# DakeQQ/Text-to-Speech-TTS-ONNX

Measured on AMD Instinct MI355X. Metric: audio_seconds_per_second, higher is better.
Workload: dtype f32

## Files before the change

include/mi355tts.h:

```cpp
#ifndef MI355TTS_H
#define MI355TTS_H

#include <stdint.h>

#ifdef __cplusplus
extern "C" {
#endif

enum { MI_F32 = 0, MI_F16 = 1, MI_BF16 = 2 };
enum { MI_HOST = 0, MI_DEVICE = 1 };
enum { MI_OK = 0, MI_EINVAL = -1, MI_EHIP = -2, MI_ENOMEM = -3, MI_ESTATE = -4 };

typedef struct mi_bigvgan mi_bigvgan;
typedef struct mi_f5 mi_f5;

int         mi_init(int device);
int         mi_device_count(void);
const char* mi_last_error(void);
const char* mi_version(void);

int64_t     mi_bigvgan_param_count(const int32_t* cfg, int n_cfg);
mi_bigvgan* mi_bigvgan_create(const int32_t* cfg, int n_cfg, const float* weights, int64_t n_weights,
                              int dtype, int device);
mi_bigvgan* mi_bigvgan_create_mem(const int32_t* cfg, int n_cfg, const float* weights, int64_t n_weights,
// ... 99 lines not shown
                                          int penalty_range, float* repeat_penality, int32_t* tokens, float* hidden, int cap,
                                          int32_t* n_out, int mem, const float* temperature, const int32_t* top_k,
                                          const float* top_p, const uint64_t* seeds);
int         mi_gpt_sample_logits(const float* logits, const float* pen, int rows, int codes, const float* temperature,
                                 const int32_t* top_k, const float* top_p, const uint64_t* seeds, const int64_t* positions,
                                 int32_t* tokens, float* u_out, float* prob_out, int mem);

int         mi_gpt_generate_beam(mi_gpt* h, int nb, const float* prompts, const int32_t* prompt_rows, const int32_t* max_new,
                                 const int32_t* stop_ids, int n_stop, float repeat_value, int penalty_range,
                                 float* repeat_penality, int num_beams, int32_t* tokens, float* hidden, int cap, int32_t* n_out,
                                 float* scores, int mem);
int         mi_gpt_beam_select(const float* logits, const float* pen, const float* prev_scores, int groups, int beams, int codes,
                               int first, int32_t* parents, int32_t* tokens, float* scores, int mem);

int         mi_gpt_generate_beam_pool(mi_gpt* h, int nb, const float* prompts, const int32_t* prompt_rows, const int32_t* max_new,
                                      const int32_t* stop_ids, int n_stop, float repeat_value, int penalty_range,
                                      const float* repeat_penality, int num_beams, float length_penalty, int early_stopping,
                                      const float* temperature, const int32_t* top_k, const float* top_p, const uint64_t* seeds,
                                      int32_t* tokens, float* hidden, int cap, int32_t* n_out, float* scores, int mem);
int         mi_gpt_beam_pool_select(const float* logits, const float* pen, const float* prev_scores, int beams, int codes, int n,
                                    int max_new, const int32_t* stop_ids, int n_stop, float* pool_scores, int32_t* pool_finished,
                                    int32_t* open, float length_penalty, int early_stopping, const float* temperature,
                                    const int32_t* top_k, const float* top_p, const uint64_t* seed, int32_t* cand, float* cand_acc,
                                    int32_t* cand_stop, int32_t* parents, int32_t* tokens, float* scores, int32_t* pool_src,
                                    int32_t* done, int mem);

int         mi_gpt_attn_decode(const float* qkv, const float* kc, const float* vc, int dtype, int heads, int max_seq, int nslots,
                               const int32_t* hist, float* out, int mem);
int         mi_gpt_attn_decode_beam(const float* qkv, const float* kc, const float* vc, int dtype, int heads, int max_seq,
                                    int nslots, const int32_t* hist, const int32_t* ndec, int beams, const int32_t* anc, float* out,
                                    int mem);
int         mi_gpt_attn_prompt(const float* qkv, const float* kc, const float* vc, int dtype, int heads, int max_seq, int hist,
                               int rows, int flag, float* out, int mem);
int         mi_gpt_attn_prompt_packed(const float* qkv, const float* kc, const float* vc, int dtype, int heads, int max_seq,
                                      int nslots, const int32_t* segs, int nseg, int total, float* out, int mem);

int         mi_gpt_linear_decode(const float* w, const float* bias, const float* x, int dtype, int n, int k, const float* ln_w,
                                 const float* ln_b, const float* pre_w, const float* pre_b, float* pre_out, const float* res,
                                 int act, int out_f32, int qkv, int hist, int max_seq, float* kc, float* vc, float* out, int mem);
int         mi_gpt_linear_batch(const float* w, const float* bias, const float* x, const float* x_dead, int dtype, int n, int k,
                                int nb, const float* res, int act, int out_f32, int qkv, const int32_t* hist, int max_seq,
                                float* kc, float* vc, float* out, int mem);
int         mi_gpt_linear_batch_rows(int nb);
int         mi_gpt_linear_decode_q8(const uint8_t* q, const float* scale, const uint8_t* zp, const float* bias, const float* x,
                                    int dtype, int n, int k, const float* ln_w, const float* ln_b, const float* pre_w,
                                    const float* pre_b, float* pre_out, const float* res, int act, int out_f32, int qkv, int hist,
                                    int max_seq, float* kc, float* vc, float* out, int mem);
int         mi_gpt_linear_batch_q8(const uint8_t* q, const float* scale, const uint8_t* zp, const float* bias, const float* x,
                                   const float* x_dead, int dtype, int n, int k, int nb, const float* res, int act, int out_f32,
                                   int qkv, const int32_t* hist, int max_seq, float* kc, float* vc, float* out, int mem);

int         mi_gpt_generate_queue(mi_gpt* h, int n, const float* prompts, const int32_t* prompt_rows, const int32_t* max_new,
                                  const int32_t* stop_ids, int n_stop, float repeat_value, int penalty_range,
                                  int32_t* tokens, float* hidden, int cap, int32_t* n_out, int mem,
                                  const float* temperature, const int32_t* top_k, const float* top_p, const uint64_t* seeds,
                                  int32_t* stats );

int         mi_gpt_queue_begin(mi_gpt* h, int n, const float* prompts, const int32_t* prompt_rows, const int32_t* max_new,
                               const int32_t* stop_ids, int n_stop, float repeat_value, int penalty_range, int32_t* tokens,
                               float* hidden, int cap, int mem, const float* temperature, const int32_t* top_k, const float* top_p,
                               const uint64_t* seeds);
int         mi_gpt_queue_advance(mi_gpt* h, int32_t* count , int32_t* done , int32_t* finished ,
                                 int32_t* stats );
int         mi_gpt_queue_end(mi_gpt* h);

int         mi_gpt_generate_queue_beam(mi_gpt* h, int n, const float* prompts, const int32_t* prompt_rows, const int32_t* max_new,
                                       const int32_t* stop_ids, int n_stop, float repeat_value, int penalty_range, int num_beams,
                                       int32_t* tokens, float* hidden, int cap, int32_t* n_out, float* scores ,
                                       int mem, int32_t* stats );
int         mi_gpt_queue_begin_beam(mi_gpt* h, int n, const float* prompts, const int32_t* prompt_rows, const int32_t* max_new,
                                    const int32_t* stop_ids, int n_stop, float repeat_value, int penalty_range, int num_beams,
                                    int32_t* tokens, float* hidden, int cap, float* scores , int mem);

int         mi_gpt_queue_schedule(int n, const int32_t* prompt_rows, const int32_t* max_new, const int32_t* lengths, int slots,
                                  int max_seq, int beams, int32_t* steps, int32_t* n_passes, int32_t* pass_of ,
                                  int32_t* unit_of );

int         mi_gpt_bench_pick(mi_gpt* h, int nb, int iters, const float* temperature, const int32_t* top_k, const float* top_p,
                              double* us);

int         mi_bench_conv_gemm(int dtype, int B, int T, int Cin, int N, int taps, int dil, int with_res, int iters,
                               double* ms);

#define MI_GEMM_PLAN_INTS 10
int         mi_conv_gemm_plan(int dtype, int B, int T, int Cin, int N, int taps, int dil, int with_res, int cus,
                              int32_t* plans , int* n_launches);

int64_t     mi_indextts_cond_param_count(const int32_t* cfg, int n_cfg);
mi_cond*    mi_indextts_cond_create(const int32_t* cfg, int n_cfg, const float* weights, int64_t n_weights, int device);
void        mi_indextts_cond_destroy(mi_cond* h);
int         mi_indextts_cond_run(mi_cond* h, const int16_t* audio, int64_t L, float* conds, float* conds_latent, float* mel,
                                 int mem);

int         mi_set_option(const char* key, int64_t value);
int         mi_get_option(const char* key, int64_t* value);
int         mi_device_pci_bus_id(int device, char* buf, int cap);

int         mi_prof_enable(int family_mask);
int         mi_prof_reset(void);
int         mi_prof_get(const char* family, double* ms, int64_t* launches, double* bytes, double* flops);
int         mi_prof_kernel_count(void);
int         mi_prof_kernel_get(int index, char* name, int name_cap, char* family, int family_cap, double* ms,
                               int64_t* launches, double* bytes, double* flops);

#ifdef __cplusplus
}
#endif
#endif
```

text-to-speech-tts-onnx_amd/csrc/capi.hip:

```cpp
#include "common.h"
#include "bigvgan.h"
#include "f5.h"
#include "gpt.h"
#include "gpt_queue.h"
#include "gpt_pool.h"
#include "cond.h"
#include <algorithm>
#include <memory>
#include <mutex>
#include <exception>

using namespace mi;

struct mi_bigvgan { BigVGAN* impl; std::mutex mu; };
struct mi_f5 { F5* impl; std::mutex mu; };
struct mi_gpt { Gpt* impl; std::mutex mu; std::unique_ptr<GptQueue> session; };
struct mi_cond { Cond* impl; std::mutex mu; };

template <typename F> static int guard(F&& f, bool exclusive = false) {
    try {
        options_init();
        std::shared_lock<std::shared_mutex> rd(option_lock(), std::defer_lock);
        std::unique_lock<std::shared_mutex> wr(option_lock(), std::defer_lock);
        if (exclusive) wr.lock(); else rd.lock();
// ... 218 lines not shown
    return guard([&] {
        MI_REQUIRE(x && w && y && B > 0 && Cin > 0 && Cout > 0 && T > 0 && k > 0 && dilation > 0 && groups > 0 && padding >= 0,
                   "mi_conv1d: bad arguments");
        unit_conv1d(x, B, Cin, T, w, bias, Cout, k, dilation, padding, groups, dtype, y);
    });
}

int mi_conv_transpose1d(const float* x, int B, int Cin, int T, const float* w, const float* bias, int Cout, int k,
                        int stride, int padding, int dtype, float* y) {
    return guard([&] {
        MI_REQUIRE(x && w && y && B > 0 && Cin > 0 && Cout > 0 && T > 0, "mi_conv_transpose1d: bad arguments");
        unit_conv_transpose1d(x, B, Cin, T, w, bias, Cout, k, stride, padding, dtype, y);
    });
}

int64_t mi_f5_param_count(const int32_t* cfg_i, int n_i, const float* cfg_f, int n_f) {
    int64_t n = -1;
    int rc = guard([&] { n = f5_param_count(parse_f5_cfg(cfg_i, n_i, cfg_f, n_f)); });
    return rc == MI_OK ? n : (int64_t)rc;
}

mi_f5* mi_f5_create(const int32_t* cfg_i, int n_i, const float* cfg_f, int n_f, const float* weights, int64_t n_weights,
                    int dtype, int device) {
    mi_f5* h = nullptr;
    int rc = guard([&] {
        MI_REQUIRE(weights != nullptr, "mi_f5_create: null weights");
        F5Cfg c = parse_f5_cfg(cfg_i, n_i, cfg_f, n_f);
        F5* impl = new F5(c, weights, n_weights, dtype, device);
        h = new mi_f5; h->impl = impl;
    });
    return rc == MI_OK ? h : nullptr;
}

mi_f5* mi_f5_create_mem(const int32_t* cfg_i, int n_i, const float* cfg_f, int n_f, const float* weights, int64_t n_weights,
                        int dtype, int device, int mem) {
    mi_f5* h = nullptr;
    int rc = guard([&] {
        MI_REQUIRE(weights != nullptr && (mem == MI_HOST || mem == MI_DEVICE), "mi_f5_create_mem: null weights / bad mem kind");
        F5Cfg c = parse_f5_cfg(cfg_i, n_i, cfg_f, n_f);
        F5* impl = new F5(c, weights, n_weights, dtype, device, mem);
        h = new mi_f5; h->impl = impl;
    });
    return rc == MI_OK ? h : nullptr;
}

void mi_f5_destroy(mi_f5* h) {
    if (!h) return;
    delete h->impl;
    delete h;
}

struct F5Recover {
    F5* e; int n;
    explicit F5Recover(F5* e_) : e(e_), n(std::uncaught_exceptions()) {}
    ~F5Recover() { if (std::uncaught_exceptions() > n) e->recover(); }
};
#define F5_CHECK(h, mem, name)                                                     \
    MI_REQUIRE((h) && (h)->impl, name ": null handle");                            \
    std::lock_guard<std::mutex> lk_((h)->mu);                                      \
    F5Recover rec_((h)->impl);                                                     \
    ArithScope arith_((h)->impl->arith);                                           \
    MI_REQUIRE((mem) == MI_HOST || (mem) == MI_DEVICE, name ": bad mem kind")

int mi_f5_tables(mi_f5* h, float* time_expand, float* delta_t) {
    return guard([&] {
        MI_REQUIRE(h && h->impl, "mi_f5_tables: null handle");
        std::lock_guard<std::mutex> lk_(h->mu);
        F5& e = *h->impl;
        if (time_expand) std::memcpy(time_expand, e.h_time_expand.data(), e.h_time_expand.size() * 4);
        if (delta_t) std::memcpy(delta_t, e.h_delta.data(), e.h_delta.size() * 4);
    });
}

int64_t mi_f5_info(mi_f5* h, const char* key) {
    int64_t v = -1;
    int rc = guard([&] {
        MI_REQUIRE(h && h->impl && key, "mi_f5_info: null handle / key");
        std::lock_guard<std::mutex> lk_(h->mu);
        F5& e = *h->impl;
        ArithScope as(e.arith);
        const std::string k(key);
        if (k == "f32_arithmetic") v = e.dtype != MI_F32 ? -1 : !gemm_x3_enabled() ? ARITH_NATIVE : (gemm_x3p_enabled() ? e.np : ARITH_BF16X3);
        else if (k == "saturation_events") v = e.sat_events;
        else if (k == "adaln_fold") v = (e.fold_built && e.cfg.ln_fold != 0) ? 1 : 0;
        else if (k == "attn_v_rows") v = attention_kv_layout(0, e.dtype, true).v_rows;
        else MI_REQUIRE(false, "mi_f5_info: unknown key");
    });
    return rc == MI_OK ? v : (int64_t)rc;
}

int mi_f5_preprocess(mi_f5* h, const int16_t* audio, int64_t L, const int32_t* text_ids, int64_t T, int64_t max_duration,
                     const float* noise_in, uint64_t seed, float* noise, float* rope_cos, float* rope_sin,
                     float* cat_mel_text, float* cat_mel_text_drop, int64_t* ref_signal_len, int mem) {
    return guard([&] {
        F5_CHECK(h, mem, "mi_f5_preprocess");
        F5& e = *h->impl;
        MI_REQUIRE(max_duration > 0 && max_duration <= e.cfg.max_len && T >= 0 && T < (1 << 20) && L > 0 && L < (1L << 31),
                   "mi_f5_preprocess: sizes");
        const int N = (int)max_duration;
        const int R = e.preprocess(1, audio, L, text_ids, (int)T, N, noise_in, seed, mem);
        hipStream_t s = e.stream;
        const size_t cd = e.cfg.cond_dim(), D = e.cfg.dim_head;
        copy_out(noise, e.d_noise.p, (size_t)N * e.cfg.mel * 4, mem, s);
        copy_out(rope_cos, e.rope_cos.p, (size_t)N * D * 4, mem, s);
        copy_out(rope_sin, e.rope_sin.p, (size_t)N * D * 4, mem, s);
        copy_out(cat_mel_text, e.d_cmt.p, (size_t)N * cd * 4, mem, s);
        copy_out(cat_mel_text_drop, e.d_cmtd.p, (size_t)N * cd * 4, mem, s);
        MI_HIP(hipStreamSynchronize(s));
        e.finish_call();
        if (ref_signal_len) *ref_signal_len = R;
    });
}

int mi_f5_transformer_step(mi_f5* h, float* noise, const float* cmt, const float* cmtd, int U, int64_t N,
                           int32_t* time_step, int fuse, int mem) {
    return guard([&] {
        F5_CHECK(h, mem, "mi_f5_transformer_step");
        MI_REQUIRE(noise && cmt && cmtd && time_step && fuse >= 1 && U >= 1 && N > 0, "mi_f5_transformer_step: bad arguments");
        F5& e = *h->impl;
        f5_run_checked(e, [&] {
            e.load_cond(noise, cmt, cmtd, U, (int)N, mem);
            e.build_cat_cond(U, (int)N);
            e.steps(U, (int)N, *time_step, fuse);
            MI_HIP(hipStreamSynchronize(e.stream));
        });
        copy_out(noise, e.d_noise.p, (size_t)U * N * e.cfg.mel * 4, mem, e.stream);
        MI_HIP(hipStreamSynchronize(e.stream));
        e.finish_call();
        *time_step += fuse;
    });
}

int mi_f5_sample(mi_f5* h, float* noise, const float* cmt, const float* cmtd, int U, int64_t N, int k0, int n_steps, int mem) {
    return guard([&] {
        F5_CHECK(h, mem, "mi_f5_sample");
        MI_REQUIRE(noise && cmt && cmtd && U >= 1 && N > 0, "mi_f5_sample: bad arguments");
        F5& e = *h->impl;
        f5_run_checked(e, [&] {
            e.load_cond(noise, cmt, cmtd, U, (int)N, mem);
            e.build_cat_cond(U, (int)N);
            e.steps(U, (int)N, k0, n_steps);
            MI_HIP(hipStreamSynchronize(e.stream));
        });
        copy_out(noise, e.d_noise.p, (size_t)U * N * e.cfg.mel * 4, mem, e.stream);
        MI_HIP(hipStreamSynchronize(e.stream));
        e.finish_call();
    });
}

int mi_f5_dit_eval(mi_f5* h, const float* noise, const float* cmt, const float* cmtd, int U, int64_t N, int k, float* pred, int mem) {
    return guard([&] {
        F5_CHECK(h, mem, "mi_f5_dit_eval");
        MI_REQUIRE(noise && cmt && cmtd && pred && U >= 1 && N > 0, "mi_f5_dit_eval: bad arguments");
        F5& e = *h->impl;
        f5_run_checked(e, [&] {
            e.load_cond(noise, cmt, cmtd, U, (int)N, mem);
            e.build_cat_cond(U, (int)N);
            e.dit_eval(U, (int)N, k);
            MI_HIP(hipStreamSynchronize(e.stream));
        });
        copy_out(pred, e.pred_rows(U, (int)N), (size_t)2 * U * N * e.cfg.mel * 4, mem, e.stream);
        MI_HIP(hipStreamSynchronize(e.stream));
        e.finish_call();
    });
}

// ... 1094 lines not shown
        const void* xd = ln_w ? (const void*)u.f32(x, k) : u.typed(x, 1, k, dtype);
        void* kd = qkv ? u.typed(kc, (long)(nc / 64), 64, dtype) : nullptr;
        void* vd = qkv ? u.typed(vc, (long)(nc / 64), 64, dtype) : nullptr;
        void* od = u.nan_out(n, odt);
        float* pd = pre_w ? (float*)u.nan_out(k, MI_F32) : nullptr;
        const int* st = u.state(&hist, 1, 1);
        launch_gpt_gemv(l, xd, u.f32(ln_w, k), u.f32(ln_b, k), u.f32(pre_w, k), u.f32(pre_b, k), pd, od, odt, act, u.f32(res, n), kd,
                        vd, st, qkv ? max_seq : 1, u.s);
        u.give(out, od, n, odt);
        if (pd) u.give(pre_out, pd, k, MI_F32);
        if (qkv) { u.give(kc, kd, nc, dtype); u.give(vc, vd, nc, dtype); }
        MI_HIP(hipStreamSynchronize(u.s));
    });
}

int mi_gpt_linear_decode(const float* w, const float* bias, const float* x, int dtype, int n, int k, const float* ln_w,
                         const float* ln_b, const float* pre_w, const float* pre_b, float* pre_out, const float* res, int act,
                         int out_f32, int qkv, int hist, int max_seq, float* kc, float* vc, float* out, int mem) {
    return linear_decode_unit("mi_gpt_linear_decode", w, LinQ8{nullptr, nullptr, nullptr}, bias, x, dtype, n, k, ln_w, ln_b, pre_w, pre_b,
                              pre_out, res, act, out_f32, qkv, hist, max_seq, kc, vc, out, mem);
}

int mi_gpt_linear_decode_q8(const uint8_t* q, const float* scale, const uint8_t* zp, const float* bias, const float* x, int dtype, int n,
                            int k, const float* ln_w, const float* ln_b, const float* pre_w, const float* pre_b, float* pre_out,
                            const float* res, int act, int out_f32, int qkv, int hist, int max_seq, float* kc, float* vc, float* out,
                            int mem) {
    if (!q) return guard([&] { MI_REQUIRE(false, "mi_gpt_linear_decode_q8: null argument"); });
    return linear_decode_unit("mi_gpt_linear_decode_q8", nullptr, LinQ8{q, scale, zp}, bias, x, dtype, n, k, ln_w, ln_b, pre_w, pre_b,
                              pre_out, res, act, out_f32, qkv, hist, max_seq, kc, vc, out, mem);
}

static int linear_batch_unit(const std::string& who, const float* w, const LinQ8& q8, const float* bias, const float* x,
                             const float* x_dead, int dtype, int n, int k, int nb, const float* res, int act, int out_f32, int qkv,
                             const int32_t* hist, int max_seq, float* kc, float* vc, float* out, int mem) {
    return guard([&] {
        LinUnit u(who, dtype, mem);
        MI_REQUIRE(x && out, who + ": null argument");
        MI_REQUIRE(nb >= 1 && nb <= GPT_MAX_BATCH, who + ": nb must be in [1, 64]");
        MI_REQUIRE(n >= 1 && n <= (1 << 20) && k >= 1 && k <= 16384, who + ": n must be in [1, 2^20], k in [1, 16384]");
        MI_REQUIRE(act == ACT_NONE || act == ACT_GELU_TANH, who + ": act must be 0 or 1 (gelu_new)");
        if (qkv) {
            MI_REQUIRE(n % 3 == 0 && n == 3 * k && k % 64 == 0, who + ": qkv needs n == 3 * k (a multiple of 3), k a multiple of 64");
            MI_REQUIRE(kc && vc && hist, who + ": qkv needs kc, vc and hist");
            MI_REQUIRE(max_seq >= 1 && max_seq <= 8192, who + ": max_seq must be in [1, 8192]");
            for (int b = 0; b < nb; ++b) MI_REQUIRE(hist[b] >= 0 && hist[b] <= max_seq, who + ": hist must be in [0, max_seq]");
        }
        const int odt = out_f32 ? MI_F32 : dtype, P = gpt_padded_rows(nb);
        const size_t sstride = qkv ? (size_t)k * max_seq : 0, nc = (size_t)nb * sstride;
        const GptLin l = lin_unit_weights(u, who, w, q8, bias, dtype, n, k);
        char* xd = (char*)u.typed(x, nb, k, dtype, P);
        const size_t row = (size_t)k * dtype_size(dtype);
        if (x_dead) {
            const float* dead = u.f32(x_dead, k);
            for (int b = nb; b < P; ++b) launch_copy2d(dead, k, xd + b * row, k, 1, k, dtype, u.s);
        } else if (P > nb) {
            MI_HIP(hipMemsetAsync(xd + nb * row, 0, (P - nb) * row, u.s));
        }
        void* kd = qkv ? u.typed(kc, (long)(nc / 64), 64, dtype) : nullptr;
        void* vd = qkv ? u.typed(vc, (long)(nc / 64), 64, dtype) : nullptr;
        void* od = u.nan_out((size_t)P * n, odt);
        const int* st = u.state(qkv ? hist : nullptr, nb, P);
        launch_gpt_gemv_b(l, xd, nb, P, od, odt, act, u.f32(res, (size_t)nb * n), kd, vd, st, qkv ? max_seq : 1, sstride, u.s);
        u.give(out, od, (size_t)P * n, odt);
        if (qkv) { u.give(kc, kd, nc, dtype); u.give(vc, vd, nc, dtype); }
        MI_HIP(hipStreamSynchronize(u.s));
    });
}

int mi_gpt_linear_batch(const float* w, const float* bias, const float* x, const float* x_dead, int dtype, int n, int k, int nb,
                        const float* res, int act, int out_f32, int qkv, const int32_t* hist, int max_seq, float* kc, float* vc,
                        float* out, int mem) {
    return linear_batch_unit("mi_gpt_linear_batch", w, LinQ8{nullptr, nullptr, nullptr}, bias, x, x_dead, dtype, n, k, nb, res, act, out_f32,
                             qkv, hist, max_seq, kc, vc, out, mem);
}

int mi_gpt_linear_batch_q8(const uint8_t* q, const float* scale, const uint8_t* zp, const float* bias, const float* x,
                           const float* x_dead, int dtype, int n, int k, int nb, const float* res, int act, int out_f32, int qkv,
                           const int32_t* hist, int max_seq, float* kc, float* vc, float* out, int mem) {
    if (!q) return guard([&] { MI_REQUIRE(false, "mi_gpt_linear_batch_q8: null argument"); });
    return linear_batch_unit("mi_gpt_linear_batch_q8", nullptr, LinQ8{q, scale, zp}, bias, x, x_dead, dtype, n, k, nb, res, act, out_f32,
                             qkv, hist, max_seq, kc, vc, out, mem);
}

extern "C++" {
enum { BG_X, BG_W, BG_BIAS, BG_OUT, BG_RES, BG_W3, BG_XP, BG_W3P, BG_SK_WS, BG_SK_FLAGS, BG_COUNT };
template <typename F> static ConvGemm bench_gemm(int dtype, int B, int T, int Cin, int N, int taps, int dil, int with_res, F&& buf) {
    const size_t es = dtype_size(dtype), nx = (size_t)B * T * Cin, nw = (size_t)N * taps * Cin, no = (size_t)B * T * N;
    ConvGemm p;
    p.dtype = dtype; p.x = buf(BG_X, nx * es); p.w = buf(BG_W, nw * es); p.bias = (const float*)buf(BG_BIAS, (size_t)N * 4); p.out = buf(BG_OUT, no * es);
    p.res = with_res ? buf(BG_RES, no * es) : nullptr;
    p.B = B; p.T_in = T; p.M = T; p.N = N; p.Cin = Cin; p.taps = taps; p.dil = dil; p.pad = (taps * dil - dil) / 2;
    p.x_bstride = (long)T * Cin; p.x_rstride = Cin; p.out_bstride = (long)T * N; p.out_rstride = N;
    p.sk_slots = 1024; p.sk_ws = (float*)buf(BG_SK_WS, (size_t)p.sk_slots * 128 * 128 * 4); p.sk_flags = (int*)buf(BG_SK_FLAGS, (size_t)p.sk_slots * 4);
    if (dtype == MI_F32 && taps == 1 && gemm_x3_enabled()) p.w3 = buf(BG_W3, (size_t)3 * nw * 2);
    if (p.w3 && gemm_x3p_enabled() && N % 128 == 0 && Cin % 32 == 0 && p.pad == 0) {
        p.np = x3p_planes();
        p.xp = buf(BG_XP, (size_t)x3p_bytes((long)B * T, Cin, p.np)); p.w3p = buf(BG_W3P, (size_t)x3p_bytes(N, Cin, p.np));
    }
    return p;
}
}

int mi_conv_gemm_plan(int dtype, int B, int T, int Cin, int N, int taps, int dil, int with_res, int cus, int32_t* plans, int* n_launches) {
    return guard([&] {
        MI_REQUIRE(plans && n_launches && (dtype == MI_F32 || dtype == MI_F16 || dtype == MI_BF16) && B > 0 && T > 0 && Cin > 0 && N > 0 && taps > 0 && dil > 0 && cus > 0,
                   "mi_conv_gemm_plan: bad arguments");
        ConvGemm p = bench_gemm(dtype, B, T, Cin, N, taps, dil, with_res, [](int which, size_t) { return (void*)(uintptr_t)(4096 * (which + 1)); });
        gemm_one_m_axis(p);
        int n = 0;
        for (;;) {
            const GemmPlan g = gemm_plan(p, cus);
            const int32_t row[MI_GEMM_PLAN_INTS] = {g.kind, g.Tm, g.Tn, g.RT, g.RC, g.lds_epi, g.use_buf, (int32_t)g.grid[0], (int32_t)g.grid[1], (int32_t)g.grid[2]};
            std::memcpy(plans + (size_t)n++ * MI_GEMM_PLAN_INTS, row, sizeof(row));
            if (!g.split_rows || n == 2) break;
            p.M = p.T_in = p.M - g.split_rows;
        }
        *n_launches = n;
    });
}

int mi_bench_conv_gemm(int dtype, int B, int T, int Cin, int N, int taps, int dil, int with_res, int iters, double* ms) {
    return guard([&] {
        MI_REQUIRE(ms && B > 0 && T > 0 && Cin > 0 && N > 0 && taps > 0 && iters > 0, "mi_bench_conv_gemm: bad arguments");
        hipStream_t s;
        MI_HIP(hipStreamCreateWithFlags(&s, hipStreamNonBlocking));
        const size_t es = dtype_size(dtype);
        const size_t nx = (size_t)B * T * Cin, nw = (size_t)N * taps * Cin, no = (size_t)B * T * N;
        DevBuf bufs[BG_COUNT];
        SkWorkspace skw;
        ConvGemm p = bench_gemm(dtype, B, T, Cin, N, taps, dil, with_res, [&](int which, size_t bytes) -> void* {
            if (which == BG_SK_WS || which == BG_SK_FLAGS) { skw.ensure(1024, s); return which == BG_SK_WS ? skw.ws.p : skw.flags.p; }
            bufs[which].ensure(bytes);
            return bufs[which].p;
        });
        DevBuf &x = bufs[BG_X], &w = bufs[BG_W], &w3p = bufs[BG_W3P];
        std::vector<float> hx(nx), hw(nw), hb(N, 0.01f);
        uint32_t st = 12345;
        auto rnd = [&]() { st = st * 1664525u + 1013904223u; return ((st >> 8) & 0xffff) / 65536.0f - 0.5f; };
        for (auto& v : hx) v = rnd();
        for (auto& v : hw) v = rnd() * 0.1f;
        if (env_first_is("MI355TTS_BENCH_ZERO", '1')) { std::fill(hx.begin(), hx.end(), 0.f); std::fill(hw.begin(), hw.end(), 0.f); }
        const int nsets = std::max(1, (int)env_int("MI355TTS_BENCH_WSETS", 1));
        upload_as(x, hx.data(), nx, dtype, s); upload_as(w, hw.data(), nw, dtype, s); upload_f32(bufs[BG_BIAS], hb.data(), N, s);
        DevBuf wsets;
        if (nsets > 1) {
            wsets.ensure((size_t)nsets * nw * es);
            for (int i = 0; i < nsets; ++i)
                MI_HIP(hipMemcpyAsync((char*)wsets.p + (size_t)i * nw * es, w.p, nw * es, hipMemcpyDeviceToDevice, s));
        }
        if (p.res) MI_HIP(hipMemsetAsync(bufs[BG_RES].p, 0, no * es, s));
        if (p.w3) split3_planes((const float*)w.p, bufs[BG_W3].p, (long)nw, s);
        if (p.xp) {
            x3p_split_rows((const float*)x.p, Cin, bufs[BG_XP].p, B * T, Cin, s, p.np);
            x3p_split_rows((const float*)w.p, Cin, w3p.p, N, Cin, s, p.np);
        }
        DevBuf w3psets;
        const size_t w3pb = p.w3p ? (size_t)x3p_bytes(N, Cin, p.np) : 0;
        if (nsets > 1 && p.w3p) {
            w3psets.ensure((size_t)nsets * w3pb);
            for (int i = 0; i < nsets; ++i) MI_HIP(hipMemcpyAsync((char*)w3psets.p + (size_t)i * w3pb, w3p.p, w3pb, hipMemcpyDeviceToDevice, s));
        }
        for (int i = 0; i < 3; ++i) launch_conv_gemm(p, s);
        hipEvent_t e0, e1;
        MI_HIP(hipEventCreate(&e0)); MI_HIP(hipEventCreate(&e1));
        MI_HIP(hipEventRecord(e0, s));
        for (int i = 0; i < iters; ++i) {
// ... 99 lines not shown
```

text-to-speech-tts-onnx_amd/csrc/common.h:

```cpp
#pragma once
#include <hip/hip_runtime.h>
#include <hip/hip_fp16.h>
#include <cstdint>
#include <cstdio>
#include <cstring>
#include <cmath>
#include <string>
#include <vector>
#include <stdexcept>
#include <map>
#include <shared_mutex>

#include "../../include/mi355tts.h"
#include "options.h"

namespace mi {

struct Error : std::runtime_error {
    int code;
    Error(int c, const std::string& m) : std::runtime_error(m), code(c) {}
};
void set_last_error(const std::string& m);

#define MI_HIP(expr)                                                                              \
// ... 38 lines not shown
    void release() { if (p) { (void)hipFree(p); p = nullptr; bytes = 0; } }
    void ensure(size_t n) {
        if (n <= bytes) return;
        release();
        MI_HIP(hipMalloc(&p, n));
        bytes = n;
    }
    template <typename T> T* as() const { return reinterpret_cast<T*>(p); }
};

inline void copy_out(void* dst, const void* src, size_t bytes, int mem, hipStream_t s) {
    if (!dst) return;
    MI_HIP(hipMemcpyAsync(dst, src, bytes, mem == MI_HOST ? hipMemcpyDeviceToHost : hipMemcpyDeviceToDevice, s));
}

void upload_as(DevBuf& dst, const float* src, size_t n, int dt, hipStream_t s);
void upload_f32(DevBuf& dst, const float* src, size_t n, hipStream_t s);
int device_cus();

struct BlobReader {
    int mem; hipStream_t s;
    std::vector<std::vector<float>> keep;
    BlobReader(int mem_, hipStream_t s_) : mem(mem_), s(s_) {}
    const float* host(const float* p, size_t n);
    void put(DevBuf& dst, const float* p, size_t n, int dt, size_t dst_off = 0);
};

struct ProfScope {
    int fam; hipStream_t s; hipEvent_t e0 = nullptr, e1 = nullptr; bool on; double bytes_ = 0, flops_ = 0;
    ProfScope(int family, hipStream_t stream, double bytes, double flops);
    ~ProfScope();
};
enum { FAM_CONV_GEMM = 0, FAM_AA = 1, FAM_CONV_POST = 2, FAM_ATTN = 3, FAM_NORM = 4, FAM_OTHER = 5, FAM_COUNT = 6 };
void prof_set_kernel(const char* expr, const char* t = nullptr, const char* to = nullptr);
void prof_kernel_suffix(const char* sfx);
template <typename T> inline const char* type_label();
template <> inline const char* type_label<float>() { return "float"; }
template <> inline const char* type_label<f16>() { return "_Float16"; }
template <> inline const char* type_label<bf16>() { return "__bf16"; }
#define MI_LAUNCH(K, T_, TO_, grid, blk, lds, s, ...)                                                  \
    do {                                                                                               \
        mi::prof_set_kernel(#K, mi::type_label<T_>(), mi::type_label<TO_>());                          \
        hipLaunchKernelGGL(K, grid, blk, lds, s, __VA_ARGS__);                                         \
    } while (0)
void prof_collect();
unsigned prof_mask();

enum Act { ACT_NONE = 0, ACT_GELU_TANH = 1, ACT_GELU_ERF = 2, ACT_MISH = 3, ACT_SILU = 4 };
enum EpiMode { EPI_PLAIN = 0, EPI_CONVT = 1, EPI_QKV_ROPE = 2 };

struct ConvGemm {
    int dtype = MI_F32;
    int out_dtype = -1;
    const void* x = nullptr;
    const void* w = nullptr;
    const float* bias = nullptr;
    void* out = nullptr;
    const void* res = nullptr;
    const float* gate = nullptr;
    long gate_bstride = 0;
    int B = 1, G = 1;
    int T_in = 0;
    int M = 0, N = 0, Cin = 0, taps = 1, dil = 1, pad = 0;
    long x_bstride = 0, x_rstride = 0;
    long out_bstride = 0, out_rstride = 0;
    long x_goff = 0;
    int act = ACT_NONE;
    float alpha = 1.f;
    int accumulate = 0;
    int epi = EPI_PLAIN;
    int u = 1, Cout = 0, padT = 0, T_out = 0;
    const float* rope_cos = nullptr; const float* rope_sin = nullptr; int heads = 0, head_dim = 0;
    const void* rope_pack = nullptr;
    void* out2 = nullptr; void* out3 = nullptr;
    int rows_per_item = 0;
    int m_off = 0;
    long v_ld = 0;
    int kv_planes = 0; long k_ld = 0;
    int v_rows = 0;
    float* sk_ws = nullptr; int* sk_flags = nullptr; int sk_slots = 0;
    const void* w3 = nullptr;
    const void* xp = nullptr; const void* w3p = nullptr; int np = 3;
    const void* gcp_w = nullptr;
    void* out_planes = nullptr;
    const float* ln_scale = nullptr; void* ln_out = nullptr; float* ln_stats_out = nullptr; int ln_out_np = 0;
    const float* ln_stats_in = nullptr; const float* ln_p = nullptr; const float* ln_c = nullptr; int ln_dim = 0; float ln_eps = 0.f;
    int ln_final = 0;
    int* sat = nullptr;
    const int* lens = nullptr; int len_mul = 1, len_add = 0;
    long bias_bstride = 0;
};
constexpr int LN_BLK = 32;
void launch_conv_gemm(const ConvGemm& p, hipStream_t s);
enum GemmKind { GEMM_NONE = 0, GEMM_DIRECT_256x32, GEMM_DIRECT_128x64, GEMM_DIRECT_128x128, GEMM_DMA64, GEMM_DMA64_PAIRS, GEMM_DMA128,
                GEMM_DMA128_RING4, GEMM_PH8, GEMM_X3P, GEMM_X3, GEMM_SK, GEMM_DMA3_192, GEMM_DMA3_256, GEMM_DMA3_128 };
struct GemmPlan {
    int kind;
    int Tm, Tn, RT, RC, use_buf, lds_epi;
    int sk_stages;
    unsigned grid[3];
    bool fold_epi;
    bool planes_out;
    int split_rows;
};
void gemm_one_m_axis(ConvGemm& p);
GemmPlan gemm_plan(const ConvGemm& p, int cus);
bool gemm_ln_fold_ok(const ConvGemm& p, int cus);
constexpr int X3P_PLANE = 128 * 32 * 2;
constexpr int X3P_CHUNK = 3 * X3P_PLANE;
__host__ __device__ inline int x3p_chunk_bytes(int np) { return np * X3P_PLANE; }
__host__ __device__ inline long x3p_slot_offset(long row, int s8, int nch, int np = 3) {
    const int r = (int)(row & 127);
    return ((row >> 7) * nch + (s8 >> 2)) * (long)(np * X3P_PLANE) + r * 64 + (((s8 & 3) ^ ((r >> 2) & 3)) << 4);
}
long x3p_bytes(long rows, long K, int np = 3);
void x3p_split_rows(const float* x, long ld, void* planes, int rows, int K, hipStream_t s, int np = 3, int* sat = nullptr);
size_t gconv_pairs_planes_bytes(int G, int taps);
void gconv_pairs_split_weights(const float* w, void* wp, int G, int taps, hipStream_t s);
size_t gconv16_image_bytes(int G, int taps);
void gconv16_build_weights(const void* w, int dtype, void* img, int G, int taps, hipStream_t s);
int x3p_planes();
bool gemm_x3p_enabled();
bool gemm_x3p_would_run(const ConvGemm& p, int cus);
bool gemm_x3p_can_write_planes(const ConvGemm& p, int cus);
struct SkWorkspace {
    DevBuf ws, flags; int slots = 0;
    void ensure(int n_slots, hipStream_t s);
    void reset(hipStream_t s);
    bool tripped() const;
    void attach(ConvGemm& g) const { g.sk_ws = ws.as<float>(); g.sk_flags = flags.as<int>(); g.sk_slots = slots; }
};

struct ArithOverride {
    int gemm_x3 = -1;
    int gemm_x3p = -1;
    int planes = -1;
    int n64_pairs = -1;
    int gconv = -1;
    int attn_x3 = -1;
    int attn_np = -1;
};
enum { ARITH_DEFAULT = -1, ARITH_NATIVE = 0, ARITH_PAIRS = 2, ARITH_BF16X3 = 3 };
ArithOverride arith_for(int kind);
ArithOverride& arith_tls();
struct ArithScope {
    ArithOverride saved;
    explicit ArithScope(const ArithOverride& a) : saved(arith_tls()) { arith_tls() = a; }
    ~ArithScope() { arith_tls() = saved; }
    ArithScope(const ArithScope&) = delete;
    ArithScope& operator=(const ArithScope&) = delete;
};

struct AAAct {
    int dtype = MI_F32;
    const void* x = nullptr; void* y = nullptr;
    const float* alpha = nullptr;
    const float* inv_beta = nullptr;
    int B = 1, T = 0, C = 0;
    int post = 0;
    const int* lens = nullptr; int len_mul = 1, len_add = 0;
};
void launch_aa_act(const AAAct& p, hipStream_t s);
const float* aa_filter_host();

struct AAConv {
    int dtype = MI_F32;
    const void* x = nullptr; const void* w = nullptr;
    const float* bias = nullptr;
    const float* snake_alpha = nullptr; const float* snake_inv_beta = nullptr;
    void* out = nullptr; const void* res = nullptr;
    int B = 1, T = 0, C = 0, k = 3, dil = 1;
    float alpha = 1.f; int accumulate = 0;
    const int* lens = nullptr; int len_mul = 1, len_add = 0;
};
void launch_aa_conv(const AAConv& p, hipStream_t s);
void split3_planes(const float* w, void* planes, long n, hipStream_t s);
bool gemm_x3_enabled();

void launch_ncl_to_nlc(const float* x, void* y, int B, int C, int T, int Cpad, int dtype, hipStream_t s);
void launch_ncl_to_nlc_len(const float* x, void* y, int B, int C, int T, int Cpad, int dtype, const int* lens, const long* offs,
                           hipStream_t s);
void launch_nlc_to_ncl(const void* x, float* y, int B, int C, int T, int dtype, hipStream_t s);
void launch_conv_post(const void* x, const float* w , float bias, int B, int T, int C, int dtype,
                      int use_tanh, float* out_f32, int16_t* out_i16, hipStream_t s);
void launch_conv_post_len(const void* x, const float* w, float bias, int B, int T, int C, int dtype, int use_tanh, float* out_f32,
                          int16_t* out_i16, const int* lens, int len_mul, int len_add, const long* offs, hipStream_t s);
void launch_conv_post_win(const void* x, const float* w, float bias, int B, int T, int C, int dtype, int use_tanh, float* out_f32,
                          int16_t* out_i16, const int* lens, int len_mul, int len_add, const long* win, hipStream_t s);

}
```

text-to-speech-tts-onnx_amd/csrc/f5.h:

```cpp
#pragma once
#include <algorithm>

#include "common.h"
#include "f5_kernels.h"

namespace mi {

struct F5Cfg {
    int dim, depth, heads, dim_head, ff_mult, mel, text_dim, vocab, conv_layers, conv_mult, pos_k, pos_g, freq_dim,
        nfe, max_len, n_fft, hop, sr, vd, vi, vlayers;
    float cfg_strength, sway;
    float score_scale = 1.f;
    int f32_arith = ARITH_DEFAULT;
    int mel_type = 0;
    int ln_fold = -1;
    int ff() const { return dim * ff_mult; }
    int nb() const { return n_fft / 2 + 1; }
    int cat_dim() const { return 2 * mel + text_dim; }
    int cond_dim() const { return mel + text_dim; }
};
F5Cfg parse_f5_cfg(const int32_t* ci, int ni, const float* cf, int nf);
int64_t f5_param_count(const F5Cfg& c);

struct Lin { DevBuf w, b, w3, w3p; int n = 0, k = 0; };

struct F5 {
    F5Cfg cfg;
    int dtype, device;
    hipStream_t stream = nullptr;

    Lin in_proj, gconv1, gconv2, proj_out;
    Lin proj_out_k; int proj_parts = 1; DevBuf pred_sum;
    const float* pred_rows(int U, int N);
    int cat_pad = 0;
    int cat_ld() const { return cfg.cat_dim() + cat_pad; }
    struct Block { Lin qkv, o, ff1, ff2; };
    std::vector<Block> blocks;
    DevBuf mod;
    long mod_ld = 0;
    DevBuf delta_t;
    DevBuf rope_cos, rope_sin;
    DevBuf rope_pack;
    std::vector<float> h_time_expand, h_delta;

    DevBuf text_emb, text_pos, stft_w, fbank;
    struct TextBlock { DevBuf dw_w, dw_b, ln_w, ln_b, grn_g, grn_b; Lin pw1, pw2; };
    std::vector<TextBlock> tblocks;

    Lin v_embed, v_head, istft;
    DevBuf v_norm_w, v_norm_b, v_fnorm_w, v_fnorm_b, wsi;
    struct VBlock { DevBuf dw_w, dw_b, n_w, n_b; Lin pw1, pw2; };
    std::vector<VBlock> vblocks;

    struct GraphEntry { hipGraphExec_t exec = nullptr; int uses = 0; };
    std::map<std::vector<int>, GraphEntry> graphs;
    bool use_graph = true;
    long graph_epoch = 0;
    void drop_graphs();
    void recover();
    void steps_eager(int U, int N, int k0, int nsteps, const int* lens = nullptr);

    SkWorkspace sk;
    DevBuf attn_ws, attn_cnt;
    long attn_ws_floats = 0, attn_cnt_n = 0;
    int ws_U = 0, ws_N = 0;
    int np = 3;
    ArithOverride arith;
    int arith_kind = ARITH_DEFAULT;
    DevBuf Ap, Ap2;
    int ap2_cols() const { return std::max(cfg.ff(), cat_ld()); }
    bool fold_built = false;
    DevBuf ApN;
    DevBuf ln_stats;
    DevBuf ln_fin;
    DevBuf ln_tab;
    long ln_ld = 0, ln_blk = 0;
    DevBuf d_sat;
    long sat_events = 0;
    void build_ln_tables(int i, DevBuf& G, DevBuf& S, DevBuf& tmpw);
    void set_arith(int kind);
    bool take_saturation();
    void finish_call();
    DevBuf d_noise, d_cmt, d_cmtd, cat, h32, hT, c1, X, Ub, qb, kb, vb, Ob, Hff, pred;
    DevBuf p_audio, p_pad, p_spec, p_mag, p_mel, p_ids, p_tid, p_err, p_tx, p_ty, p_ty2, p_ss;
    std::vector<float> h_noise;
    DevBuf v_h, v_z, v_z2, v_s, v_c, v_fr, v_outf, v_outi;

    F5(const F5Cfg& c, const float* w, int64_t nw, int dt, int dev, int mem = MI_HOST);
    ~F5();
    void ensure_workspace(int U, int N);
    void gemm(int dt, const void* x, long xb, long xr, int K, const Lin& L, void* out, int odt, long ob, long orr,
              int B, int M, int act = ACT_NONE, const void* res = nullptr, const float* gate = nullptr);
    int preprocess(int U, const int16_t* audio, long L, const int32_t* text_ids, int T, int N,
                   const float* noise_in, uint64_t seed, int mem);
    void stft(const int16_t* audio_dev, int U, long L, int pad = -1);
    void check_text_ids();
    void load_cond(const float* noise, const float* cmt, const float* cmtd, int U, int N, int mem);
    void build_cat_cond(int U, int N);
    void dit_eval(int U, int N, int k, const int* lens = nullptr);
    void steps(int U, int N, int k0, int nsteps, const int* lens = nullptr);
    DevBuf d_len;
    std::vector<int> h_len;
    int ref_frames(long L) const;
    const int* set_lengths(int U, const int* lens);
    void zero_pad_rows_cond(int U, int Nmax, const int* lens);
    void preprocess_ragged(int U, const int16_t* audio, const long* L, const int32_t* text_ids, const int* T, const int* Ns, int Nmax,
                           const float* noise_in, uint64_t seed, int mem, int* R);
    long decode(const float* denoised_dev, int U, int N, int R, float* out_f, int16_t* out_i);
};

}
```

text-to-speech-tts-onnx_amd/csrc/f5.hip:

```cpp
#include "f5.h"

namespace mi {

static int rup(int a, int b) { return (a + b - 1) / b * b; }

F5Cfg parse_f5_cfg(const int32_t* ci, int ni, const float* cf, int nf) {
    MI_REQUIRE(ci && ni >= 21 && ni <= 24 && cf && (nf == 2 || nf == 3),
               "f5 cfg: expected 21 ints (+ up to 3 optional: fp32 arithmetic, mel type, AdaLN fold) + 2 floats (+ the optional attention score scale)");
    F5Cfg c;
    int i = 0;
    c.dim = ci[i++]; c.depth = ci[i++]; c.heads = ci[i++]; c.dim_head = ci[i++]; c.ff_mult = ci[i++]; c.mel = ci[i++];
    c.text_dim = ci[i++]; c.vocab = ci[i++]; c.conv_layers = ci[i++]; c.conv_mult = ci[i++]; c.pos_k = ci[i++];
    c.pos_g = ci[i++]; c.freq_dim = ci[i++]; c.nfe = ci[i++]; c.max_len = ci[i++]; c.n_fft = ci[i++]; c.hop = ci[i++];
    c.sr = ci[i++]; c.vd = ci[i++]; c.vi = ci[i++]; c.vlayers = ci[i++];
    if (ni > 21) c.f32_arith = ci[21];
    if (ni > 22) c.mel_type = ci[22];
    if (ni > 23) c.ln_fold = ci[23];
    MI_REQUIRE(c.f32_arith == ARITH_DEFAULT || c.f32_arith == ARITH_NATIVE || c.f32_arith == ARITH_PAIRS || c.f32_arith == ARITH_BF16X3,
               "f5 cfg: fp32 arithmetic is -1 (process default), 0 (native fp32 MFMA), 2 (fp16 pairs) or 3 (three bf16 planes)");
    MI_REQUIRE((c.mel_type == 0 || c.mel_type == 1) && c.ln_fold >= -1 && c.ln_fold <= 1, "f5 cfg: mel type is 0 (vocos) or 1 (bigvgan); AdaLN fold is -1, 0 or 1");
    c.cfg_strength = cf[0]; c.sway = cf[1];
    if (nf == 3) { c.score_scale = cf[2]; MI_REQUIRE(c.score_scale > 0.f && c.score_scale <= 1e4f, "f5 cfg: attention score scale"); }
    MI_REQUIRE(c.dim == c.heads * c.dim_head, "f5 cfg: dim != heads*dim_head");
    MI_REQUIRE(c.dim_head == 64, "f5: the attention kernel is built for head_dim 64");
// ... 302 lines not shown
        for (int i = 0; i < c.mel + 2; ++i) {
            const double m = m_min + (m_max - m_min) * i / (c.mel + 1);
            fpts[i] = 700.0 * (std::pow(10.0, m / 2595.0) - 1.0);
        }
        for (int k = 0; k < nb && c.mel_type == 0; ++k) {
            const double fr = (double)(c.sr / 2) * k / (nb - 1);
            for (int m = 0; m < c.mel; ++m) {
                const double down = (fr - fpts[m]) / (fpts[m + 1] - fpts[m]);
                const double up = (fpts[m + 2] - fr) / (fpts[m + 2] - fpts[m + 1]);
                fb[(size_t)m * ldm + k] = (float)std::max(0.0, std::min(down, up));
            }
        }
        upload_f32(fbank, fb.data(), fb.size(), s);
        const int kp = rup(2 * nb, 4);
        std::vector<float> ib((size_t)nf * kp, 0.f);
        for (int n = 0; n < nf; ++n)
            for (int k = 0; k < nb; ++k) {
                const double sc = ((k == 0 || k == nb - 1) ? 1.0 : 2.0) / nf * ((double)c.hop / nf) * (double)win[n];
                const double ang = 2.0 * M_PI * (double)k * (double)n / nf;
                ib[(size_t)n * kp + k] = (float)(sc * std::cos(ang));
                ib[(size_t)n * kp + nb + k] = (float)(sc * -std::sin(ang));
            }
        istft.n = nf; istft.k = kp;
        upload_f32(istft.w, ib.data(), ib.size(), s);
        const size_t wl = (size_t)nf + (size_t)c.hop * (c.max_len - 1);
        std::vector<float> ws(wl, 0.f);
        float wmax = 0.f;
        for (int n = 0; n < nf; ++n) wmax = std::max(wmax, fabsf(win[n]));
        std::vector<float> wsq(nf);
        for (int n = 0; n < nf; ++n) { const float wn = win[n] / wmax; wsq[n] = wn * wn; }
        for (int i = 0; i < c.max_len; ++i)
            for (int n = 0; n < nf; ++n) ws[(size_t)i * c.hop + n] += wsq[n];
        for (size_t i = 0; i < wl; ++i) ws[i] = (float)nf / (ws[i] * (float)c.hop + 1e-7f);
        upload_f32(wsi, ws.data(), wl, s);
    }
    {
        const int vd = c.vd, vi = c.vi;
        const size_t ewn = (size_t)vd * c.mel * 7;
        const float* ew = R.host(take(ewn), ewn); const float* eb = R.host(take(vd), vd);
        auto re = relayout(ew, vd, c.mel, 7);
        up_lin(v_embed, re.data(), eb, vd, c.mel * 7, MI_F32, s);
        R.put(v_norm_w, take(vd), vd, MI_F32); R.put(v_norm_b, take(vd), vd, MI_F32);
        vblocks.resize(c.vlayers);
        for (auto& vb_ : vblocks) {
            R.put(vb_.dw_w, take((size_t)vd * 7), (size_t)vd * 7, MI_F32); R.put(vb_.dw_b, take(vd), vd, MI_F32);
            R.put(vb_.n_w, take(vd), vd, MI_F32); R.put(vb_.n_b, take(vd), vd, MI_F32);
            const float* w1 = take((size_t)vi * vd); const float* b1 = take(vi);
            put_lin(R, vb_.pw1, w1, b1, vi, vd, MI_F32);
            const float* w2 = take((size_t)vd * vi); const float* b2 = take(vd);
            put_lin(R, vb_.pw2, w2, b2, vd, vi, MI_F32);
        }
        R.put(v_fnorm_w, take(vd), vd, MI_F32); R.put(v_fnorm_b, take(vd), vd, MI_F32);
        const float* hw = take((size_t)(c.n_fft + 2) * vd); const float* hb = take(c.n_fft + 2);
        put_lin(R, v_head, hw, hb, c.n_fft + 2, vd, MI_F32);
    }
    MI_HIP(hipStreamSynchronize(s));
    MI_REQUIRE(p - w == nw, "f5: weight walk mismatch");
}

F5::~F5() {
    drop_graphs();
    if (stream) (void)hipStreamDestroy(stream);
}

void F5::set_arith(int kind) {
    arith_kind = kind;
    arith = arith_for(kind);
    ArithScope sc(arith);
    np = x3p_planes();
    drop_graphs();
    if (dtype != MI_F32) return;
    const bool planes = gemm_x3p_enabled();
    auto build_planes = [&](Lin* L) {
        if (!planes || L->n % 128 != 0 || L->k % 32 != 0) { L->w3p.release(); return; }
        L->w3p.ensure((size_t)x3p_bytes(L->n, L->k, np));
        x3p_split_rows(L->w.as<float>(), L->k, L->w3p.p, L->n, L->k, stream, np);
    };
    for (Block& bk : blocks)
        for (Lin* L : {&bk.qkv, &bk.o, &bk.ff1, &bk.ff2}) build_planes(L);
    build_planes(&in_proj);
    if (ws_U > 0) {
        const long rows = (long)2 * ws_U * ws_N;
        Ap.ensure((size_t)x3p_bytes(rows, cfg.dim, np)); Ap2.ensure((size_t)x3p_bytes(rows, ap2_cols(), np)); ApN.ensure((size_t)x3p_bytes(rows, cfg.dim, np));
    }
    MI_HIP(hipStreamSynchronize(stream));
}

void F5::build_ln_tables(int i, DevBuf& G, DevBuf& S, DevBuf& tmpw) {
    const int d = cfg.dim, ff = cfg.ff(), steps = cfg.nfe;
    Block& bk = blocks[i];
    float* tab = ln_tab.as<float>() + (size_t)i * ln_blk;
    auto run = [&](const Lin& L, long col_shift, long col_scale, float* out_p, float* out_c) {
        launch_ln_gather(mod.as<float>(), mod_ld, (long)i * 6 * d + col_scale, (long)i * 6 * d + col_shift, G.as<float>(), S.as<float>(), steps, d, stream);
        const float* w32 = L.w.as<float>();
        if (dtype != MI_F32) { launch_cast_to_f32(L.w.p, dtype, tmpw.as<float>(), (long)L.n * L.k, stream); w32 = tmpw.as<float>(); }
        ConvGemm g;
        g.dtype = MI_F32; g.x = G.p; g.w = w32; g.bias = nullptr; g.out = out_p;
        g.B = 1; g.T_in = steps; g.M = steps; g.N = L.n; g.Cin = d; g.x_rstride = d; g.x_bstride = (long)steps * d;
        g.out_rstride = ln_ld; g.out_bstride = (long)steps * ln_ld;
        launch_conv_gemm(g, stream);
        g.x = S.p; g.bias = L.b.as<float>(); g.out = out_c;
        launch_conv_gemm(g, stream);
        MI_HIP(hipStreamSynchronize(stream));
    };
    run(bk.qkv, 0, d, tab, tab + 3 * d);
    run(bk.ff1, 3 * d, 4 * d, tab + 6 * d, tab + 6 * d + ff);
}

bool F5::take_saturation() {
    if (!d_sat.p) return false;
    int flag = 0;
    MI_HIP(hipMemcpy(&flag, d_sat.p, 4, hipMemcpyDeviceToHost));
    if (!flag) return false;
    MI_HIP(hipMemset(d_sat.p, 0, 4));
    return true;
}

void F5::finish_call() {
    check_text_ids();
}

void F5::ensure_workspace(int U, int N) {
    if (U <= ws_U && N <= ws_N) return;
    drop_graphs();
    const int Um = std::max(U, ws_U), Nm = std::max(N, ws_N);
    const F5Cfg& c = cfg;
    const size_t es = dtype_size(dtype);
    const size_t rows = (size_t)2 * Um * Nm;
    sk.ensure(1024, stream);
    {
        if (ATTN_WS_TILES > attn_cnt_n) {
            attn_ws_floats = ATTN_WS_TILES * ATTN_MAX_SLICES * ATTN_SLOT_SPLIT;
            attn_ws.ensure((size_t)attn_ws_floats * 4);
            attn_cnt.ensure((size_t)ATTN_WS_TILES * 4);
            MI_HIP(hipMemsetAsync(attn_cnt.p, 0, (size_t)ATTN_WS_TILES * 4, stream));
            attn_cnt_n = ATTN_WS_TILES;
        }
    }
    d_noise.ensure((size_t)Um * Nm * c.mel * 4);
    d_cmt.ensure((size_t)Um * Nm * c.cond_dim() * 4);
    d_cmtd.ensure((size_t)Um * Nm * c.cond_dim() * 4);
    if (rows * cat_ld() * es > cat.bytes) {
        cat.ensure(rows * cat_ld() * es);
        if (cat_ld() != c.cat_dim()) MI_HIP(hipMemsetAsync(cat.p, 0, cat.bytes, stream));
    }
    h32.ensure(rows * c.dim * 4); hT.ensure(rows * c.dim * es); c1.ensure(rows * c.dim * es);
    X.ensure(rows * c.dim * 4); Ub.ensure(rows * c.dim * es);
    qb.ensure(rows * c.dim * es); Ob.ensure(rows * c.dim * es);
    {
        const size_t keypad = (size_t)(Nm + 63) / 64 * 64;
        size_t kbytes = rows * c.dim * es, vbytes = (size_t)2 * Um * (size_t)(Nm + 8) * c.dim * es;
        if (dtype == MI_F32) { kbytes = std::max(kbytes, (size_t)2 * Um * keypad * c.dim * 6); vbytes = std::max(vbytes, (size_t)2 * Um * keypad * c.dim * 6); }
        if (kbytes > kb.bytes) { kb.ensure(kbytes); MI_HIP(hipMemsetAsync(kb.p, 0, kbytes, stream)); }
        if (vbytes > vb.bytes) { vb.ensure(vbytes); MI_HIP(hipMemsetAsync(vb.p, 0, vbytes, stream)); }
    }
    Hff.ensure(rows * c.ff() * es);
    if (dtype == MI_F32) {
        Ap.ensure((size_t)x3p_bytes((long)rows, c.dim, np)); Ap2.ensure((size_t)x3p_bytes((long)rows, ap2_cols(), np));
        if (fold_built) ApN.ensure((size_t)x3p_bytes((long)rows, c.dim, np));
    }
    if (fold_built) { ln_stats.ensure((rows + 128) * (size_t)(c.dim / LN_BLK) * 2 * 4); if (dtype != MI_F32) ln_fin.ensure((rows + 128) * 8); }
    pred.ensure(rows * c.mel * 4 * proj_parts);
    if (proj_parts > 1) pred_sum.ensure(rows * c.mel * 4);
    const int ti = c.text_dim * c.conv_mult;
    p_ids.ensure((size_t)Um * Nm * 4);
    p_tx.ensure((size_t)2 * Um * Nm * c.text_dim * 4); p_ty.ensure((size_t)2 * Um * Nm * c.text_dim * 4);
    p_ty2.ensure((size_t)2 * Um * Nm * ti * 4); p_ss.ensure((size_t)2 * Um * ti * 4);
    const size_t fr = (size_t)Um * Nm;
    v_h.ensure(fr * c.vd * 4); v_z.ensure(fr * c.vd * 4); v_z2.ensure(fr * c.vi * 4);
    v_s.ensure(fr * (c.n_fft + 2) * 4); v_c.ensure(fr * istft.k * 4); v_fr.ensure(fr * c.n_fft * 4);
    v_outf.ensure(fr * c.hop * 4); v_outi.ensure(fr * c.hop * 2);
    ws_U = Um; ws_N = Nm;
}

void F5::gemm(int dt, const void* x, long xb, long xr, int K, const Lin& L, void* out, int odt, long ob, long orr, int B,
              int M, int act, const void* res, const float* gate) {
    ConvGemm g;
    g.dtype = dt; g.out_dtype = odt; g.x = x; g.w = L.w.p; g.w3 = L.w3.p; g.bias = L.b.p ? L.b.as<float>() : nullptr; g.out = out;
    g.res = res; g.gate = gate; g.gate_bstride = 0;
    g.B = B; g.T_in = M; g.M = M; g.N = L.n; g.Cin = K; g.taps = 1;
    g.x_bstride = xb; g.x_rstride = xr; g.out_bstride = ob; g.out_rstride = orr; g.act = act;
    g.sat = d_sat.as<int>();
    sk.attach(g);
    if (B > 1 && xb == (long)M * xr && ob == (long)M * orr) {
        g.B = 1; g.T_in = B * M; g.M = B * M;
    }
    if (dt == MI_F32 && L.w3p.p && g.B == 1 && Ap.p && gemm_x3p_enabled()) {
        DevBuf& ab = K <= cfg.dim ? Ap : Ap2;
        g.xp = ab.p; g.w3p = L.w3p.p; g.np = np;
        if (gemm_x3p_would_run(g, device_cus())) {
            MI_REQUIRE(x3p_bytes(g.M, K, np) <= (long)ab.bytes, "F5::gemm: the panel planes of the rows do not fit their buffer");
            x3p_split_rows((const float*)x, xr, const_cast<void*>(g.xp), g.M, K, stream, np, d_sat.as<int>());
        } else {
            g.xp = nullptr; g.w3p = nullptr;
        }
    }
    launch_conv_gemm(g, stream);
}

static inline uint64_t splitmix64(uint64_t x) {
    x += 0x9E3779B97F4A7C15ull;
    uint64_t z = x;
    z = (z ^ (z >> 30)) * 0xBF58476D1CE4E5B9ull;
    z = (z ^ (z >> 27)) * 0x94D049BB133111EBull;
    return z ^ (z >> 31);
}
static void host_normal(float* out, size_t n, uint64_t seed) {
    for (size_t i = 0; i < n; ++i) {
        const uint64_t a = splitmix64(seed * 0x2545F4914F6CDD1Dull + 2 * i), b = splitmix64(seed * 0x2545F4914F6CDD1Dull + 2 * i + 1);
        const double u1 = ((double)(a >> 11) + 1.0) / 9007199254740993.0, u2 = (double)(b >> 11) / 9007199254740992.0;
        out[i] = (float)(std::sqrt(-2.0 * std::log(u1)) * std::cos(2.0 * M_PI * u2));
    }
}

int F5::preprocess(int U, const int16_t* audio, long L, const int32_t* text_ids, int T, int N,
                   const float* noise_in, uint64_t seed, int mem) {
    const F5Cfg& c = cfg;
    MI_REQUIRE(audio && text_ids && U >= 1 && L >= c.n_fft / 2 + 1 && T >= 0, "f5_preprocess: bad arguments");
    const int mel_pad = c.mel_type == 1 ? (c.n_fft - c.hop) / 2 : c.n_fft / 2;
    MI_REQUIRE(L + 2 * mel_pad >= c.n_fft && L > mel_pad, "f5_preprocess: audio shorter than one STFT frame");
    const int R = (int)((L + 2 * mel_pad - c.n_fft) / c.hop) + 1;
    MI_REQUIRE(N >= R && N >= T && N <= c.max_len, "f5_preprocess: max_duration must be >= ref frames, >= text length and <= max_signal_length");
    if (mem == MI_HOST)
        for (long i = 0; i < (long)U * T; ++i) {
            const long id = (long)text_ids[i] + 1;
            MI_REQUIRE(id >= 0 && id <= c.vocab, "f5_preprocess: text id out of range");
        }
    MI_HIP(hipSetDevice(device));
    ensure_workspace(U, N);
    hipStream_t s = stream;
    const int nf = c.n_fft, nb = c.nb(), ldm = rup(nb, 8), cd = c.cond_dim();
    const long Lp = L + nf;
    p_audio.ensure((size_t)U * L * 2); p_pad.ensure((size_t)U * Lp * 4 + 64);
    p_spec.ensure((size_t)U * R * 2 * nb * 4); p_mag.ensure((size_t)U * R * ldm * 4); p_mel.ensure((size_t)U * R * c.mel * 4);
    p_tid.ensure((size_t)U * std::max(T, 1) * 4); p_err.ensure(4);
    const int16_t* da = audio;
    const int32_t* dt_ids = text_ids;
    if (mem == MI_HOST) {
        MI_HIP(hipMemcpyAsync(p_audio.p, audio, (size_t)U * L * 2, hipMemcpyHostToDevice, s));
        da = p_audio.as<int16_t>();
        if (T > 0) MI_HIP(hipMemcpyAsync(p_tid.p, text_ids, (size_t)U * T * 4, hipMemcpyHostToDevice, s));
        dt_ids = p_tid.as<int32_t>();
    }
    MI_HIP(hipMemsetAsync(p_err.p, 0, 4, s));
    stft(da, U, L, mel_pad);
    launch_spec_mag(p_spec.as<float>(), p_mag.as<float>(), U * R, nb, ldm, c.mel_type == 1 ? 1e-9f : 0.f, s);
    {
        ConvGemm g;
        g.dtype = MI_F32; g.x = p_mag.p; g.w = fbank.p; g.out = p_mel.p;
        g.B = 1; g.T_in = U * R; g.M = U * R; g.N = c.mel; g.Cin = ldm; g.x_rstride = ldm; g.out_rstride = c.mel;
        launch_conv_gemm(g, s);
    }
    launch_logmel(p_mel.as<float>(), d_cmt.as<float>(), d_cmtd.as<float>(), U, N, R, c.mel, cd, s);
    const int td = c.text_dim, ti = td * c.conv_mult;
    int* dids = p_ids.as<int>();
    launch_text_ids(dt_ids, dids, U, T, N, c.vocab, p_err.as<int>(), s);
    float* tx = p_tx.as<float>(); float* ty = p_ty.as<float>(); float* ty2 = p_ty2.as<float>();
    launch_text_gather(dids, text_emb.as<float>(), text_pos.as<float>(), tx, U, N, td, s);
    const int B2 = 2 * U;
    for (auto& tb : tblocks) {
        launch_dwconv7(tx, ty, tb.dw_w.as<float>(), tb.dw_b.as<float>(), B2, N, td, s);
        launch_rownorm(NORM_LN_AFFINE, ty, ty, MI_F32, tb.ln_w.as<float>(), tb.ln_b.as<float>(), (long)B2 * N, td, 1e-6f, s);
        gemm(MI_F32, ty, (long)N * td, td, td, tb.pw1, ty2, MI_F32, (long)N * ti, ti, B2, N, ACT_GELU_ERF);
        launch_grn(ty2, p_ss.as<float>(), tb.grn_g.as<float>(), tb.grn_b.as<float>(), B2, N, ti, s);
        gemm(MI_F32, ty2, (long)N * ti, ti, ti, tb.pw2, tx, MI_F32, (long)N * td, td, B2, N, ACT_NONE, tx);
        launch_mask_rows(dids, tx, B2, N, td, s);
    }
    for (int u = 0; u < U; ++u) {
        launch_copy2d(tx + (size_t)(2 * u) * N * td, td, d_cmt.as<float>() + (size_t)u * N * cd + c.mel, cd, N, td, MI_F32, s);
        launch_copy2d(tx + (size_t)(2 * u + 1) * N * td, td, d_cmtd.as<float>() + (size_t)u * N * cd + c.mel, cd, N, td, MI_F32, s);
    }
    const size_t nn = (size_t)N * c.mel;
    if (noise_in) {
        MI_HIP(hipMemcpyAsync(d_noise.p, noise_in, (size_t)U * nn * 4, mem == MI_HOST ? hipMemcpyHostToDevice : hipMemcpyDeviceToDevice, s));
    } else {
        h_noise.resize((size_t)U * nn);
        for (int u = 0; u < U; ++u) host_normal(h_noise.data() + (size_t)u * nn, nn, seed + (uint64_t)u);
        MI_HIP(hipMemcpyAsync(d_noise.p, h_noise.data(), h_noise.size() * 4, hipMemcpyHostToDevice, s));
    }
    return R;
}

void F5::stft(const int16_t* audio_dev, int U, long L, int pad) {
    const F5Cfg& c = cfg;
    if (pad < 0) pad = c.n_fft / 2;
    const int nf = c.n_fft, nb = c.nb(), R = (int)((L + 2 * pad - nf) / c.hop) + 1;
    const long Lp = L + 2 * pad;
    launch_pad_reflect(audio_dev, p_pad.as<float>(), U, L, pad, stream);
    ConvGemm g;
    g.dtype = MI_F32; g.x = p_pad.p; g.w = stft_w.p; g.out = p_spec.p;
    g.B = U; g.T_in = R; g.M = R; g.N = 2 * nb; g.Cin = nf; g.x_rstride = c.hop; g.x_bstride = Lp;
    g.out_rstride = 2 * nb; g.out_bstride = (long)R * 2 * nb;
    launch_conv_gemm(g, stream);
}

void F5::check_text_ids() {
    if (sk.tripped()) {
        recover();
        MI_REQUIRE(false, "f5: a split-tile hand-off timed out on the device (workspace reset; results of this call discarded)");
    }
    if (!p_err.p) return;
    int flag = 0;
    MI_HIP(hipMemcpy(&flag, p_err.p, 4, hipMemcpyDeviceToHost));
    if (flag != 0) {
        MI_HIP(hipMemset(p_err.p, 0, 4));
        MI_REQUIRE(false, "f5_preprocess: text id out of range");
    }
}

void F5::load_cond(const float* noise, const float* cmt, const float* cmtd, int U, int N, int mem) {
    const F5Cfg& c = cfg;
    MI_REQUIRE(U > 0 && N > 0 && N <= c.max_len, "f5: bad batch / length");
    MI_HIP(hipSetDevice(device));
    ensure_workspace(U, N);
    const hipMemcpyKind kind = mem == MI_HOST ? hipMemcpyHostToDevice : hipMemcpyDeviceToDevice;
    if (noise && noise != d_noise.p) MI_HIP(hipMemcpyAsync(d_noise.p, noise, (size_t)U * N * c.mel * 4, kind, stream));
    if (cmt && cmt != d_cmt.p) MI_HIP(hipMemcpyAsync(d_cmt.p, cmt, (size_t)U * N * c.cond_dim() * 4, kind, stream));
    if (cmtd && cmtd != d_cmtd.p) MI_HIP(hipMemcpyAsync(d_cmtd.p, cmtd, (size_t)U * N * c.cond_dim() * 4, kind, stream));
}

void F5::build_cat_cond(int U, int N) {
    const F5Cfg& c = cfg;
    const size_t es = dtype_size(dtype);
    const int cd = c.cond_dim(), ld = cat_ld();
    for (int u = 0; u < U; ++u)
        for (int br = 0; br < 2; ++br) {
            const float* src = (br == 0 ? d_cmt.as<float>() : d_cmtd.as<float>()) + (size_t)u * N * cd;
            char* dst = (char*)cat.p + ((size_t)(2 * u + br) * N * ld + c.mel) * es;
            launch_copy2d(src, cd, dst, ld, N, cd, dtype, stream);
        }
}

void F5::dit_eval(int U, int N, int k, const int* lens) {
    const F5Cfg& c = cfg;
    MI_REQUIRE(k >= 0 && k < c.nfe, "f5: time step out of range");
    hipStream_t s = stream;
    const int B = 2 * U, d = c.dim, ld = cat_ld(), ff = c.ff(), H = c.heads, D = c.dim_head;
    const long rows = (long)B * N;
    const float* modk = mod.as<float>() + (size_t)k * mod_ld;
    launch_cat_noise(d_noise.as<float>(), cat.p, U, N, c.mel, ld, dtype, s);
    gemm(dtype, cat.p, (long)N * ld, ld, ld, in_proj, h32.p, MI_F32, (long)N * d, d, B, N);
    const void* hin = h32.p;
    if (dtype != MI_F32) { launch_copy2d(h32.as<float>(), d, hT.p, d, rows, d, dtype, s); hin = hT.p; }
    const long row_bytes = (long)d * (long)dtype_size(dtype);
    if (lens) launch_zero_pad_rows(const_cast<void*>(hin), row_bytes, B, N, lens, 2, s);
    {
        ConvGemm g;
        g.dtype = dtype; g.x = hin; g.w = gconv1.w.p; g.bias = gconv1.b.as<float>(); g.out = c1.p;
        g.B = B; g.G = c.pos_g; g.T_in = N; g.M = N; g.N = d / c.pos_g; g.Cin = d / c.pos_g; g.taps = c.pos_k; g.pad = c.pos_k / 2;
        g.x_bstride = (long)N * d; g.x_rstride = d; g.x_goff = d / c.pos_g; g.out_bstride = (long)N * d; g.out_rstride = d;
        g.act = ACT_MISH; g.sat = d_sat.as<int>(); g.gcp_w = gconv1.w3p.p;
        launch_conv_gemm(g, s);
        if (lens) launch_zero_pad_rows(c1.p, row_bytes, B, N, lens, 2, s);
        g.x = c1.p; g.w = gconv2.w.p; g.bias = gconv2.b.as<float>(); g.out = X.p; g.out_dtype = MI_F32; g.res = h32.p; g.gcp_w = gconv2.w3p.p;
        launch_conv_gemm(g, s);
    }
    const bool f32 = dtype == MI_F32;
    auto lin = [&](const Lin& L, int K, int odt, void* out) {
        ConvGemm g;
        g.dtype = dtype; g.out_dtype = odt; g.w = L.w.p; g.w3 = L.w3.p; g.bias = L.b.p ? L.b.as<float>() : nullptr; g.out = out;
        g.B = 1; g.T_in = (int)rows; g.M = (int)rows; g.N = L.n; g.Cin = K; g.taps = 1;
        g.x_bstride = rows * K; g.x_rstride = K; g.out_bstride = rows * L.n; g.out_rstride = L.n;
        g.sat = d_sat.as<int>();
        sk.attach(g);
        return g;
    };
    auto with_planes = [&](ConvGemm& g, const Lin& L, const void* xp) { g.xp = xp; g.w3p = L.w3p.p; g.np = np; };
    auto attn_plan = [&](bool presplit) {
        return attention_plan(B * H, H, N, dtype, presplit, lens != nullptr, cfg.score_scale != 1.f ? cfg.score_scale : 0.f, attn_ws_floats, attn_cnt_n);
    };
    AttnPlan ap = attn_plan(false);
    auto qkv_gemm = [&](const Block& bk) {
        ConvGemm g = lin(bk.qkv, d, -1, qb.p);
        g.x = Ub.p; g.out2 = kb.p; g.out3 = vb.p; g.rows_per_item = N;
        g.epi = EPI_QKV_ROPE; g.rope_cos = rope_cos.as<float>(); g.rope_sin = rope_sin.as<float>(); g.rope_pack = rope_pack.p; g.heads = H; g.head_dim = D;
        g.kv_planes = ap.kv.kv_planes; g.k_ld = ap.kv.k_ld; g.v_ld = ap.kv.v_ld; g.v_rows = ap.kv.v_rows;
        return g;
    };
    bool planes = false, fold = false;
    const int cus = device_cus();
    {
        const Block& b0 = blocks[0];
        ConvGemm gq = qkv_gemm(b0);
        ConvGemm go = lin(b0.o, d, MI_F32, X.p); go.x = Ob.p; go.res = X.p; go.gate = modk;
        ConvGemm g1 = lin(b0.ff1, d, dtype, Hff.p); g1.x = Ub.p; g1.act = ACT_GELU_TANH;
        ConvGemm g2 = lin(b0.ff2, ff, MI_F32, X.p); g2.x = Hff.p; g2.res = X.p; g2.gate = modk;
        if (f32 && Ap.p && gemm_x3p_enabled() && b0.qkv.w3p.p && b0.o.w3p.p && b0.ff1.w3p.p && b0.ff2.w3p.p && ap.o_planes) {
            with_planes(gq, b0.qkv, Ap.p); with_planes(go, b0.o, Ap.p); with_planes(g1, b0.ff1, Ap.p); with_planes(g2, b0.ff2, Ap2.p);
            planes = gemm_x3p_would_run(gq, cus) && gemm_x3p_would_run(go, cus) && gemm_x3p_can_write_planes(g1, cus) && gemm_x3p_would_run(g2, cus);
        }
        if (fold_built && cfg.ln_fold != 0 && (planes || !f32) && (!f32 || ApN.p) && ln_stats.p && (f32 || ln_fin.p)) {
            if (f32) { with_planes(gq, b0.qkv, ApN.p); with_planes(g1, b0.ff1, ApN.p); }
            fold = gemm_ln_fold_ok(gq, cus) && gemm_ln_fold_ok(go, cus) && gemm_ln_fold_ok(g1, cus) && gemm_ln_fold_ok(g2, cus);
        }
    }
    if (f32 && (fold || planes)) ap = attn_plan(true);
    void* const attn_planes = f32 && (fold || planes) ? Ap.p : nullptr;
    auto attention = [&] {
        launch_attention(ap, qb.p, kb.p, vb.p, Ob.p, attn_planes, np, attn_ws.as<float>(), attn_cnt.as<int>(), lens, s);
    };
    float* stats = ln_stats.as<float>();
    const float* lnk = fold ? ln_tab.as<float>() + (size_t)k * ln_ld : nullptr;
    const bool fin = fold && !f32;
    auto finalize = [&] { if (fin) launch_ln_finalize(stats, ln_fin.as<float>(), rows, d, 1e-6f, s); };
    auto consume = [&](ConvGemm& g, const float* p, const float* c_) {
        g.bias = nullptr; g.ln_p = p; g.ln_c = c_;
        g.ln_stats_in = fin ? ln_fin.as<float>() : stats; g.ln_final = fin ? 1 : 0; g.ln_dim = d; g.ln_eps = 1e-6f;
    };
    auto produce = [&](ConvGemm& g, const float* scale) { g.ln_scale = scale; g.ln_out = f32 ? ApN.p : Ub.p; g.ln_out_np = np; g.ln_stats_out = stats; };
    if (fold) {
        launch_ln_prologue(X.as<float>(), f32 ? ApN.p : Ub.p, dtype, np, stats, modk + d, rows, d, d_sat.as<int>(), s);
        finalize();
    }
    const void* normed = fold ? ApN.p : Ap.p;
    auto layer = [&](ConvGemm& g, const Lin& L, const void* xp, const char* left) {
        if (f32) { with_planes(g, L, xp); MI_REQUIRE(gemm_x3p_would_run(g, cus), left); }
        launch_conv_gemm(g, s);
    };
    for (int i = 0; i < c.depth; ++i) {
        const Block& bk = blocks[i];
        const float* m = modk + (size_t)i * 6 * d;
        if (fold || planes) {
            const float* lt = fold ? lnk + (size_t)i * ln_blk : nullptr;
            const bool last = i + 1 == c.depth;
            if (!fold) launch_rownorm_x3p(X.as<float>(), Ap.p, m + d, m, rows, d, 1e-6f, s, np, d_sat.as<int>());
            {
                ConvGemm g = qkv_gemm(bk);
                if (fold) consume(g, lt, lt + 3 * d);
                layer(g, bk.qkv, normed, "f5: the QKV layer left the panel-plane kernel between the decision and the launch");
            }
            attention();
            {
                ConvGemm g = lin(bk.o, d, MI_F32, X.p);
                g.x = Ob.p; g.res = X.p; g.gate = m + 2 * d;
                if (fold) produce(g, m + 4 * d);
                layer(g, bk.o, Ap.p, "f5: the O projection left the panel-plane kernel between the decision and the launch");
                finalize();
            }
            if (!fold) launch_rownorm_x3p(X.as<float>(), Ap.p, m + 4 * d, m + 3 * d, rows, d, 1e-6f, s, np, d_sat.as<int>());
            {
                ConvGemm g = lin(bk.ff1, d, dtype, Hff.p);
                g.x = Ub.p; g.act = ACT_GELU_TANH;
                if (f32) g.out_planes = Ap2.p;
                if (fold) consume(g, lt + 6 * d, lt + 6 * d + ff);
                layer(g, bk.ff1, normed, "f5: the FF1 layer left the panel-plane kernel between the decision and the launch");
            }
            {
                ConvGemm g = lin(bk.ff2, ff, MI_F32, X.p);
                g.x = Hff.p; g.res = X.p; g.gate = m + 5 * d;
                if (fold && !last) produce(g, m + 6 * d + d);
                layer(g, bk.ff2, Ap2.p, "f5: the FF2 layer left the panel-plane kernel between the decision and the launch");
                if (!last) finalize();
            }
            continue;
        }
        launch_rownorm(NORM_LN_MOD, X.as<float>(), Ub.p, dtype, m + d, m, rows, d, 1e-6f, s);
        {
            ConvGemm g = qkv_gemm(bk);
            g.x_bstride = (long)B * N * d;
            launch_conv_gemm(g, s);
        }
        attention();
        gemm(dtype, Ob.p, (long)N * d, d, d, bk.o, X.p, MI_F32, (long)N * d, d, B, N, ACT_NONE, X.p, m + 2 * d);
        launch_rownorm(NORM_LN_MOD, X.as<float>(), Ub.p, dtype, m + 4 * d, m + 3 * d, rows, d, 1e-6f, s);
        gemm(dtype, Ub.p, (long)N * d, d, d, bk.ff1, Hff.p, dtype, (long)N * ff, ff, B, N, ACT_GELU_TANH);
        gemm(dtype, Hff.p, (long)N * ff, ff, ff, bk.ff2, X.p, MI_F32, (long)N * d, d, B, N, ACT_NONE, X.p, m + 5 * d);
    }
    const float* mf = modk + (size_t)c.depth * 6 * d;
    launch_rownorm(NORM_LN_MOD, X.as<float>(), Ub.p, dtype, mf, mf + d, rows, d, 1e-6f, s);
    if (proj_parts > 1) {
        ConvGemm g;
        g.dtype = dtype; g.out_dtype = MI_F32; g.x = Ub.p; g.w = proj_out_k.w.p; g.bias = proj_out_k.b.as<float>(); g.out = pred.p;
        g.B = 1; g.G = proj_parts; g.T_in = (int)rows; g.M = (int)rows; g.N = c.mel; g.Cin = d / proj_parts; g.taps = 1;
        g.x_bstride = rows * d; g.x_rstride = d; g.x_goff = d / proj_parts;
        g.out_bstride = rows * proj_parts * c.mel; g.out_rstride = (long)proj_parts * c.mel;
        launch_conv_gemm(g, s);
    } else
        gemm(dtype, Ub.p, (long)N * d, d, d, proj_out, pred.p, MI_F32, (long)N * c.mel, c.mel, B, N);
}

const float* F5::pred_rows(int U, int N) {
    if (proj_parts <= 1) return pred.as<float>();
    launch_sum_parts(pred.as<float>(), pred_sum.as<float>(), (long)2 * U * N, cfg.mel, proj_parts, stream);
    return pred_sum.as<float>();
}

void F5::steps_eager(int U, int N, int k0, int nsteps, const int* lens) {
    for (int k = k0; k < k0 + nsteps; ++k) {
        dit_eval(U, N, k, lens);
        if (lens)
            launch_cfg_update_len(d_noise.as<float>(), pred.as<float>(), U, N, cfg.mel, cfg.cfg_strength, delta_t.as<float>(), k, lens, stream,
                                  proj_parts);
        else
            launch_cfg_update(d_noise.as<float>(), pred.as<float>(), U, N, cfg.mel, cfg.cfg_strength, delta_t.as<float>(), k, stream, proj_parts);
    }
}

void F5::drop_graphs() {
    for (auto& kv : graphs)
        if (kv.second.exec) (void)hipGraphExecDestroy(kv.second.exec);
    graphs.clear();
}

void F5::recover() {
    (void)hipSetDevice(device);
    (void)hipStreamSynchronize(stream);
    (void)hipGetLastError();
    drop_graphs();
    sk.reset(stream);
    if (attn_cnt.p && attn_cnt_n > 0) {
        (void)hipMemsetAsync(attn_cnt.p, 0, (size_t)attn_cnt_n * 4, stream);
        (void)hipStreamSynchronize(stream);
    }
    if (p_err.p) (void)hipMemset(p_err.p, 0, 4);
    if (d_sat.p) (void)hipMemset(d_sat.p, 0, 4);
}

void F5::steps(int U, int N, int k0, int nsteps, const int* lens) {
    MI_REQUIRE(k0 >= 0 && nsteps >= 0 && k0 + nsteps <= cfg.nfe - 1, "f5: step range exceeds the NFE grid");
    MI_REQUIRE(!lens || lens == d_len.p, "f5: ragged steps read the handle's length table");
    if (!use_graph || prof_mask() != 0 || nsteps < 2) { steps_eager(U, N, k0, nsteps, lens); return; }
    if (graph_epoch != option_epoch()) { drop_graphs(); graph_epoch = option_epoch(); }
    GraphEntry& e = graphs[{U, N, k0, nsteps, lens ? 1 : 0}];
    if (e.exec) { MI_HIP(hipGraphLaunch(e.exec, stream)); return; }
    if (e.uses++ == 0) { steps_eager(U, N, k0, nsteps, lens); return; }
    hipGraph_t graph = nullptr;
    MI_HIP(hipStreamBeginCapture(stream, hipStreamCaptureModeThreadLocal));
    try {
        steps_eager(U, N, k0, nsteps, lens);
    } catch (...) {
        (void)hipStreamEndCapture(stream, &graph);
        if (graph) (void)hipGraphDestroy(graph);
        throw;
    }
    MI_HIP(hipStreamEndCapture(stream, &graph));
    hipError_t err = hipGraphInstantiate(&e.exec, graph, nullptr, nullptr, 0);
    (void)hipGraphDestroy(graph);
    if (err != hipSuccess) { e.exec = nullptr; use_graph = false; steps_eager(U, N, k0, nsteps, lens); return; }
    MI_HIP(hipGraphLaunch(e.exec, stream));
}

int F5::ref_frames(long L) const {
    const int mel_pad = cfg.mel_type == 1 ? (cfg.n_fft - cfg.hop) / 2 : cfg.n_fft / 2;
    return (int)((L + 2 * mel_pad - cfg.n_fft) / cfg.hop) + 1;
}

const int* F5::set_lengths(int U, const int* lens) {
    h_len.assign(lens, lens + U);
    if ((size_t)U * 4 > d_len.bytes) { drop_graphs(); d_len.ensure((size_t)std::max(U, 8) * 4); }
    MI_HIP(hipMemcpyAsync(d_len.p, h_len.data(), (size_t)U * 4, hipMemcpyHostToDevice, stream));
    return d_len.as<int>();
}

void F5::zero_pad_rows_cond(int U, int Nmax, const int* lens) {
    const size_t cd = cfg.cond_dim(), M = cfg.mel;
    for (int u = 0; u < U; ++u) {
        const size_t n = (size_t)lens[u], pad = (size_t)(Nmax - lens[u]);
        if (pad == 0) continue;
        MI_HIP(hipMemsetAsync(d_noise.as<float>() + ((size_t)u * Nmax + n) * M, 0, pad * M * 4, stream));
        MI_HIP(hipMemsetAsync(d_cmt.as<float>() + ((size_t)u * Nmax + n) * cd, 0, pad * cd * 4, stream));
        MI_HIP(hipMemsetAsync(d_cmtd.as<float>() + ((size_t)u * Nmax + n) * cd, 0, pad * cd * 4, stream));
    }
}

void F5::preprocess_ragged(int U, const int16_t* audio, const long* L, const int32_t* text_ids, const int* T, const int* Ns, int Nmax,
                           const float* noise_in, uint64_t seed, int mem, int* R) {
    const size_t M = cfg.mel, cd = cfg.cond_dim();
    MI_HIP(hipSetDevice(device));
    ensure_workspace(U, Nmax);
    std::vector<long> a_off(U + 1, 0), t_off(U + 1, 0), n_off(U + 1, 0);
    for (int u = 0; u < U; ++u) { a_off[u + 1] = a_off[u] + L[u]; t_off[u + 1] = t_off[u] + T[u]; n_off[u + 1] = n_off[u] + Ns[u]; }
    const hipMemcpyKind d2d = hipMemcpyDeviceToDevice;
    for (int u = U - 1; u >= 0; --u) {
        const int N = Ns[u];
        R[u] = preprocess(1, audio + a_off[u], L[u], text_ids + t_off[u], T[u], N, noise_in ? noise_in + (size_t)n_off[u] * M : nullptr,
                          seed + (uint64_t)u, mem);
        if (u > 0) {
            MI_HIP(hipMemcpyAsync(d_noise.as<float>() + (size_t)u * Nmax * M, d_noise.p, (size_t)N * M * 4, d2d, stream));
            MI_HIP(hipMemcpyAsync(d_cmt.as<float>() + (size_t)u * Nmax * cd, d_cmt.p, (size_t)N * cd * 4, d2d, stream));
            MI_HIP(hipMemcpyAsync(d_cmtd.as<float>() + (size_t)u * Nmax * cd, d_cmtd.p, (size_t)N * cd * 4, d2d, stream));
        }
        MI_HIP(hipStreamSynchronize(stream));
        check_text_ids();
    }
    zero_pad_rows_cond(U, Nmax, Ns);
}

long F5::decode(const float* den, int U, int N, int R, float* out_f, int16_t* out_i) {
    const F5Cfg& c = cfg;
    const int F = N - R;
    MI_REQUIRE(R >= 0 && F >= 1, "f5_decode: max_duration leaves no generated frame");
    if (F == 1) return 0;
    hipStream_t s = stream;
    const int vd = c.vd, vi = c.vi, nf = c.n_fft, nb = c.nb();
    const long rows = (long)U * F;
    float* h = v_h.as<float>(); float* z = v_z.as<float>(); float* z2 = v_z2.as<float>();
    {
        ConvGemm g;
        g.dtype = MI_F32; g.x = den + (size_t)R * c.mel; g.w = v_embed.w.p; g.bias = v_embed.b.as<float>(); g.out = h;
        g.B = U; g.T_in = F; g.M = F; g.N = vd; g.Cin = c.mel; g.taps = 7; g.pad = 3;
        g.x_bstride = (long)N * c.mel; g.x_rstride = c.mel; g.out_bstride = (long)F * vd; g.out_rstride = vd;
        launch_conv_gemm(g, s);
    }
    launch_rownorm(NORM_L2, h, h, MI_F32, v_norm_w.as<float>(), v_norm_b.as<float>(), rows, vd, 0.f, s);
    for (auto& vbk : vblocks) {
        launch_dwconv7(h, z, vbk.dw_w.as<float>(), vbk.dw_b.as<float>(), U, F, vd, s);
        launch_rownorm(NORM_L2, z, z, MI_F32, vbk.n_w.as<float>(), vbk.n_b.as<float>(), rows, vd, 0.f, s);
        gemm(MI_F32, z, (long)F * vd, vd, vd, vbk.pw1, z2, MI_F32, (long)F * vi, vi, U, F, ACT_GELU_ERF);
        gemm(MI_F32, z2, (long)F * vi, vi, vi, vbk.pw2, h, MI_F32, (long)F * vd, vd, U, F, ACT_NONE, h);
    }
    launch_rownorm(NORM_L2, h, z, MI_F32, v_fnorm_w.as<float>(), v_fnorm_b.as<float>(), rows, vd, 0.f, s);
    gemm(MI_F32, z, (long)F * vd, vd, vd, v_head, v_s.p, MI_F32, (long)F * 2 * nb, 2 * nb, U, F);
    launch_vocos_head(v_s.as<float>(), v_c.as<float>(), rows, nb, istft.k, s);
    gemm(MI_F32, v_c.p, (long)F * istft.k, istft.k, istft.k, istft, v_fr.p, MI_F32, (long)F * nf, nf, U, F);
    launch_istft_ola(v_fr.as<float>(), wsi.as<float>(), U, F, nf, c.hop, out_f, out_i, s);
    return (long)(F - 1) * c.hop;
}

}
```

text-to-speech-tts-onnx_amd/csrc/f5_kernels.h:

```cpp
#pragma once
#include "common.h"

namespace mi {

enum { NORM_LN_MOD = 0, NORM_LN_AFFINE = 1, NORM_L2 = 2 };
void launch_rownorm(int mode, const float* x, void* y, int out_dtype, const float* a, const float* b, long rows, int D,
                    float eps, hipStream_t s);
void launch_rownorm_len(int mode, const float* x, void* y, int out_dtype, const float* a, const float* b, int items, int Fmax, int D,
                        float eps, const int* lens, const long* offs, hipStream_t s);
void launch_rownorm_x3p(const float* x, void* planes, const float* a, const float* b, long rows, int D, float eps, hipStream_t s,
                        int np = 3, int* sat = nullptr);
void launch_ln_prologue(const float* x, void* aout, int a_dtype, int np, float* stats, const float* scale, long rows, int D, int* sat,
                        hipStream_t s);
void launch_ln_finalize(const float* partials, float* fin, long rows, int D, float eps, hipStream_t s);
void launch_ln_gather(const float* mod, long mod_ld, long col_scale, long col_shift, float* G, float* S, int steps, int D, hipStream_t s);
void launch_cast_to_f32(const void* src, int dtype, float* dst, long n, hipStream_t s);
void launch_absmax(const float* x, long n, unsigned* out_bits, hipStream_t s);
void launch_dwconv7(const float* x, float* y, const float* w, const float* bias, int B, int T, int C, hipStream_t s);
void launch_grn(float* y, float* ss_scratch, const float* gamma, const float* beta, int B, int T, int C, hipStream_t s);
void launch_text_gather(const int* ids, const float* emb, const float* pos, float* out, int U, int N, int C, hipStream_t s);
void launch_text_ids(const int32_t* in, int* out, int U, int T, int N, int vocab, int* err, hipStream_t s);
void launch_mask_rows(const int* ids, float* x, int V, int N, int C, hipStream_t s);
void launch_copy2d(const float* src, long lds_, void* dst, long ldd, long rows, int cols, int out_dtype, hipStream_t s);
void launch_pad_reflect(const int16_t* a, float* out, int U, long L, int half, hipStream_t s);
void launch_spec_mag(const float* spec, float* mag, int F, int nb, int ldm, float eps, hipStream_t s);
void launch_logmel(const float* melraw, float* cmt, float* cmtd, int U, int N, int R, int M, int ld, hipStream_t s);
void launch_vocos_head(const float* sp, float* c, long rows, int nb, int ldc, hipStream_t s);
void launch_istft_ola(const float* frames, const float* wsi, int U, int F, int nfft, int hop, float* out_f,
                      int16_t* out_i, hipStream_t s);
void launch_cat_noise(const float* noise, void* cat, int U, int N, int M, int ldc, int dtype, hipStream_t s);
void launch_cfg_update(float* noise, const float* pred, int U, int N, int M, float cfg, const float* dt, int k, hipStream_t s, int parts = 1);
void launch_cfg_update_len(float* noise, const float* pred, int U, int N, int M, float cfg, const float* dt, int k, const int* len,
                           hipStream_t s, int parts = 1);
void launch_zero_pad_rows(void* x, long row_bytes, int items, int N, const int* len, int per, hipStream_t s);
void launch_sum_parts(const float* in, float* out, long rows, int M, int parts, hipStream_t s);

struct AttnKvLayout {
    int kv_planes = 0;
    long k_ld = 0;
    long v_ld = 0;
    int v_rows = 0;
};
AttnKvLayout attention_kv_layout(int N, int dtype, bool caller_can_presplit_kv);
enum AttnForm {
    ATTN_F32 = 0, ATTN_F32_QK_X3 = 2, ATTN_X3F = 4, ATTN_X3F_BF16X3 = 6, ATTN_X3F_PAIRS = 8,
    ATTN_X3F_PAIRS_SLICED = 10,
    ATTN_F16 = 11, ATTN_F16_REF = 13, ATTN_BF16 = 15, ATTN_FORMS = 17
};
constexpr int ATTN_TILE = 128, ATTN_TILE_SPLIT = 64, ATTN_STAGE = 64, ATTN_MAX_SLICES = 4;
constexpr long ATTN_SLOT_GROUP = 32 * 64 + 64 * 2, ATTN_SLOT_SPLIT = 2 * ATTN_SLOT_GROUP, ATTN_SLOT = 4 * ATTN_SLOT_GROUP;
constexpr long ATTN_WS_TILES = 2048;
struct AttnPlan {
    AttnKvLayout kv;
    bool o_planes = false;
    int form = ATTN_F32;
    bool varlen = false;
    int BH = 0, H = 0, N = 0, dtype = MI_F32;
    unsigned grid[3] = {1, 1, 1};
    int cut[3] = {0, 0, 0};
    int xmap = 0;
    float sscale = 1.f;
    const char* label = "";
};
AttnPlan attention_plan(int BH, int H, int N, int dtype, bool caller_can_presplit_kv, bool has_lens, float ref_fp16_scale, long ws_floats,
                        long cnt_n);
void launch_attention(const AttnPlan& plan, const void* q, const void* k, const void* v, void* o, void* o_planes, int o_np, float* ws,
                      int* cnt, const int* lens, hipStream_t s);

}
```

text-to-speech-tts-onnx_amd/csrc/f5_kernels.hip:

```cpp
#include <type_traits>
#include "wave_reduce.h"
#include "common.h"
#include "f5_kernels.h"
#include "x3_split.h"

namespace mi {


template <typename TO, int MAXV, bool LENS = false>
__global__ __launch_bounds__(256) void rownorm_kernel(const float* __restrict__ x, TO* __restrict__ y,
                                                      const float* __restrict__ a, const float* __restrict__ b,
                                                      long rows, int D, int mode, float eps, const int* lens = nullptr,
                                                      const long* offs = nullptr, int Fmax = 0) {
    const int lane = threadIdx.x & 63;
    const long row = (long)blockIdx.x * 4 + (threadIdx.x >> 6);
    if (row >= rows) return;
    const float* xr = x + row * D;
    if constexpr (LENS) {
        const int it = __builtin_amdgcn_readfirstlane((int)(row / Fmax)), t = (int)(row - (long)it * Fmax);
        if (t >= __builtin_amdgcn_readfirstlane(lens[it])) {
            TO* yz = y + row * D;
#pragma unroll
            for (int i = 0; i < MAXV; ++i) {
                const int c = (i * 64 + lane) * 4;
// ... 485 lines not shown
    if (i >= (long)N * M) return;
    const int n = (int)(i / M), m = (int)(i - (long)n * M);
    const long u = blockIdx.y;
    melraw += u * R * M; cmt += u * N * ld; cmtd += u * N * ld;
    cmt[(long)n * ld + m] = n < R ? logf(fmaxf(melraw[(long)n * M + m], 1e-5f)) : 0.f;
    cmtd[(long)n * ld + m] = 0.f;
}
void launch_logmel(const float* melraw, float* cmt, float* cmtd, int U, int N, int R, int M, int ld, hipStream_t s) {
    const long n = (long)N * M;
    hipLaunchKernelGGL(logmel_kernel, dim3((unsigned)((n + 255) / 256), U), dim3(256), 0, s, melraw, cmt, cmtd, N, R, M, ld);
    MI_HIP(hipGetLastError());
}

__global__ __launch_bounds__(256) void vocos_head_kernel(const float* __restrict__ sp, float* __restrict__ c, long rows, int nb, int ldc) {
    const long i = (long)blockIdx.x * 256 + threadIdx.x;
    if (i >= rows * ldc) return;
    const long r = i / ldc;
    const int k = (int)(i - r * ldc);
    float v = 0.f;
    if (k < 2 * nb) {
        const int kk = k < nb ? k : k - nb;
        const float mag = fminf(expf(sp[r * 2 * nb + kk]), 100.0f);
        const float ph = sp[r * 2 * nb + nb + kk];
        v = k < nb ? mag * cosf(ph) : mag * sinf(ph);
    }
    c[i] = v;
}
void launch_vocos_head(const float* sp, float* c, long rows, int nb, int ldc, hipStream_t s) {
    const long n = rows * ldc;
    hipLaunchKernelGGL(vocos_head_kernel, dim3((unsigned)((n + 255) / 256)), dim3(256), 0, s, sp, c, rows, nb, ldc);
    MI_HIP(hipGetLastError());
}

__global__ __launch_bounds__(256) void istft_ola_kernel(const float* __restrict__ fr, const float* __restrict__ wsi,
                                                        int F, int nfft, int hop, float* __restrict__ out_f,
                                                        int16_t* __restrict__ out_i) {
    const long len = (long)(F - 1) * hop;
    const long i = (long)blockIdx.x * 256 + threadIdx.x;
    const int u = blockIdx.y;
    if (i >= len) return;
    const long t = i + nfft / 2;
    long f1 = t / hop;
    if (f1 > F - 1) f1 = F - 1;
    long f0 = (t - nfft + hop) / hop;
    if (t - nfft + 1 <= 0) f0 = 0;
    const float* fb = fr + (long)u * F * nfft;
    float acc = 0.f;
    for (long f = f0; f <= f1; ++f) acc += fb[f * nfft + (t - f * hop)];
    float v = acc * wsi[t];
    if (out_f) out_f[(long)u * len + i] = v;
    if (out_i) {
        v = fminf(fmaxf(v, -1.0f), 1.0f) * 32767.0f;
        out_i[(long)u * len + i] = (int16_t)v;
    }
}
void launch_istft_ola(const float* frames, const float* wsi, int U, int F, int nfft, int hop, float* out_f,
                      int16_t* out_i, hipStream_t s) {
    const long len = (long)(F - 1) * hop;
    if (len <= 0) return;
    hipLaunchKernelGGL(istft_ola_kernel, dim3((unsigned)((len + 255) / 256), U), dim3(256), 0, s, frames, wsi, F, nfft, hop, out_f, out_i);
    MI_HIP(hipGetLastError());
}

template <typename T>
__global__ __launch_bounds__(256) void cat_noise_kernel(const float* __restrict__ noise, T* __restrict__ cat, long UN, int M, int ldc, int N) {
    const long i = (long)blockIdx.x * 256 + threadIdx.x;
    if (i >= UN * M) return;
    const long un = i / M;
    const int m = (int)(i - un * M);
    const long u = un / N, n = un - u * N;
    const T v = from_f32<T>(noise[i]);
    cat[((2 * u) * N + n) * ldc + m] = v;
    cat[((2 * u + 1) * N + n) * ldc + m] = v;
}
void launch_cat_noise(const float* noise, void* cat, int U, int N, int M, int ldc, int dtype, hipStream_t s) {
    const long n = (long)U * N * M;
    dim3 grid((unsigned)((n + 255) / 256));
    if (dtype == MI_F32) hipLaunchKernelGGL(cat_noise_kernel<float>, grid, dim3(256), 0, s, noise, (float*)cat, (long)U * N, M, ldc, N);
    else if (dtype == MI_F16) hipLaunchKernelGGL(cat_noise_kernel<f16>, grid, dim3(256), 0, s, noise, (f16*)cat, (long)U * N, M, ldc, N);
    else hipLaunchKernelGGL(cat_noise_kernel<bf16>, grid, dim3(256), 0, s, noise, (bf16*)cat, (long)U * N, M, ldc, N);
    MI_HIP(hipGetLastError());
}

__global__ __launch_bounds__(256) void cfg_update_kernel(float* __restrict__ noise, const float* __restrict__ pred,
                                                         long NM, int M, int parts, long total, float cfg, const float* __restrict__ dt, int k) {
    const long i = (long)blockIdx.x * 256 + threadIdx.x;
    if (i >= total) return;
    const long u = i / NM, r = i - u * NM;
    const long n = r / M; const int m = (int)(r - n * M);
    const float* c = pred + ((2 * u) * NM + n * M) * parts + m;
    const float* un = c + NM * parts;
    float pc = c[0], pu = un[0];
    for (int q = 1; q < parts; ++q) { pc += c[(long)q * M]; pu += un[(long)q * M]; }
    noise[i] += (pc + (pc - pu) * cfg) * dt[k];
}
void launch_cfg_update(float* noise, const float* pred, int U, int N, int M, float cfg, const float* dt, int k, hipStream_t s, int parts) {
    const long total = (long)U * N * M;
    hipLaunchKernelGGL(cfg_update_kernel, dim3((unsigned)((total + 255) / 256)), dim3(256), 0, s, noise, pred, (long)N * M, M, parts, total, cfg, dt, k);
    MI_HIP(hipGetLastError());
}

__global__ __launch_bounds__(256) void cfg_update_len_kernel(float* __restrict__ noise, const float* __restrict__ pred,
                                                             long NM, int M, int parts, long total, float cfg, const float* __restrict__ dt,
                                                             int k, const int* __restrict__ len) {
    const long i = (long)blockIdx.x * 256 + threadIdx.x;
    if (i >= total) return;
    const long u = i / NM, r = i - u * NM;
    const long n = r / M; const int m = (int)(r - n * M);
    if (n >= len[u]) { noise[i] = 0.f; return; }
    const float* c = pred + ((2 * u) * NM + n * M) * parts + m;
    const float* un = c + NM * parts;
    float pc = c[0], pu = un[0];
    for (int q = 1; q < parts; ++q) { pc += c[(long)q * M]; pu += un[(long)q * M]; }
    noise[i] += (pc + (pc - pu) * cfg) * dt[k];
}
void launch_cfg_update_len(float* noise, const float* pred, int U, int N, int M, float cfg, const float* dt, int k, const int* len,
                           hipStream_t s, int parts) {
    const long total = (long)U * N * M;
    hipLaunchKernelGGL(cfg_update_len_kernel, dim3((unsigned)((total + 255) / 256)), dim3(256), 0, s, noise, pred, (long)N * M, M, parts,
                       total, cfg, dt, k, len);
    MI_HIP(hipGetLastError());
}

__global__ __launch_bounds__(256) void zero_pad_rows_kernel(uint4* __restrict__ x, int row_vec, int N, const int* __restrict__ len, int per) {
    const int item = (int)blockIdx.y, r0 = (int)blockIdx.x * 8;
    const int live = len[item / per];
    if (r0 + 8 <= live) return;
    const int first = r0 > live ? r0 : live, last = r0 + 8 < N ? r0 + 8 : N;
    uint4* base = x + (long)item * N * row_vec;
    for (long i = (long)first * row_vec + threadIdx.x; i < (long)last * row_vec; i += 256) base[i] = make_uint4(0, 0, 0, 0);
}
void launch_zero_pad_rows(void* x, long row_bytes, int items, int N, const int* len, int per, hipStream_t s) {
    MI_REQUIRE(row_bytes % 16 == 0 && items > 0 && N > 0 && per > 0, "zero_pad_rows: bad shape");
    hipLaunchKernelGGL(zero_pad_rows_kernel, dim3((unsigned)((N + 7) / 8), (unsigned)items), dim3(256), 0, s, (uint4*)x, (int)(row_bytes / 16),
                       N, len, per);
    MI_HIP(hipGetLastError());
}

__global__ __launch_bounds__(256) void sum_parts_kernel(const float* __restrict__ in, float* __restrict__ out, long total, int M, int parts) {
    const long i = (long)blockIdx.x * 256 + threadIdx.x;
    if (i >= total) return;
    const long row = i / M; const int m = (int)(i - row * M);
    const float* p = in + row * M * parts + m;
    float v = p[0];
    for (int q = 1; q < parts; ++q) v += p[(long)q * M];
    out[i] = v;
}
void launch_sum_parts(const float* in, float* out, long rows, int M, int parts, hipStream_t s) {
    const long total = rows * M;
    hipLaunchKernelGGL(sum_parts_kernel, dim3((unsigned)((total + 255) / 256)), dim3(256), 0, s, in, out, total, M, parts);
    MI_HIP(hipGetLastError());
}

}
```

text-to-speech-tts-onnx_amd/csrc/gconv16.hip:

```cpp
#include "common.h"
#include "gemm_epilogue.h"
#include "mfma.h"
#include "lds_dma.h"
#include <algorithm>

namespace mi {

constexpr int GC16_C = 64, GC16_S = GC16_C + 8, GC16_WTAP = GC16_C * GC16_S;

size_t gconv16_image_bytes(int G, int taps) { return (size_t)G * ((taps + 1) / 2 * 2) * GC16_WTAP * 2; }

template <typename T>
__global__ __launch_bounds__(256) void gconv16_image_kernel(const T* __restrict__ w, T* __restrict__ img, int G, int taps, int tp) {
    const long i = (long)blockIdx.x * 256 + threadIdx.x;
    const long n = (long)G * taps * GC16_C * 8;
    if (i >= n) return;
    const int c8 = (int)(i & 7), co = (int)((i >> 3) & 63);
    const long gt = i >> 9;
    const int t = (int)(gt % taps), g = (int)(gt / taps);
    *reinterpret_cast<uint4*>(img + ((long)g * tp + t) * GC16_WTAP + co * GC16_S + c8 * 8) =
        *reinterpret_cast<const uint4*>(w + (((long)g * GC16_C + co) * taps + t) * GC16_C + c8 * 8);
}

void gconv16_build_weights(const void* w, int dtype, void* img, int G, int taps, hipStream_t s) {
// ... 59 lines not shown
            const int t = t_base + row;
            uint4 u = make_uint4(0, 0, 0, 0);
            if (t >= 0 && t < p.T_in) u = *reinterpret_cast<const uint4*>(xb + (long)t * p.x_rstride + c8 * 8);
            *reinterpret_cast<uint4*>(AP + row * S + c8 * 8) = u;
        }
    }
    wait_vm<0>();
    __syncthreads();

    f32x16 acc[TM];
#pragma unroll
    for (int i = 0; i < TM; ++i)
#pragma unroll
        for (int r = 0; r < 16; ++r) acc[i][r] = 0.f;
    for (int j = 0; j < npair; ++j) {
        if (j + 1 < npair) wdma(j + 1);
        const int t = 2 * j + kg;
        if (t < p.taps) {
            const T* b_row = WS + ((j & 1) * 2 + kg) * GC16_WTAP + (wn * 32 + lr) * S + hi * 8;
            const T* a_row = AP + (wm * WM + lr + t) * S + hi * 8;
#pragma unroll
            for (int ks = 0; ks < 4; ++ks) {
                const FR bf = *reinterpret_cast<const FR*>(b_row + ks * 16);
                FR af[TM];
#pragma unroll
                for (int i = 0; i < TM; ++i) af[i] = *reinterpret_cast<const FR*>(a_row + i * 32 * S + ks * 16);
#pragma unroll
                for (int i = 0; i < TM; ++i) acc[i] = MF::mma(af[i], bf, acc[i]);
            }
        }
        wait_vm<0>();
        __syncthreads();
    }
    auto at = [&](int i, int r) -> float& { return OUT[(wm * WM + i * 32 + (r & 3) + 8 * (r >> 2) + 4 * hi) * GC16_C + wn * 32 + lr]; };
    if (kg == 1) {
#pragma unroll
        for (int i = 0; i < TM; ++i)
#pragma unroll
            for (int r = 0; r < 16; ++r) at(i, r) = acc[i][r];
    }
    __syncthreads();
    if (kg == 0) {
#pragma unroll
        for (int i = 0; i < TM; ++i)
#pragma unroll
            for (int r = 0; r < 16; ++r) at(i, r) = acc[i][r] + at(i, r);
    }
    __syncthreads();
    {
        TO* ob = (TO*)p.out + (long)b * p.out_bstride + (long)g * GC16_C;
        const TO* rb = p.res ? (const TO*)p.res + (long)b * p.out_bstride + (long)g * GC16_C : nullptr;
        const float* bias = p.bias ? p.bias + g * GC16_C : nullptr;
        for (int v = tid; v < BM * 16; v += 512) {
            const int row = v >> 4, c4 = v & 15;
            const int m = m0 + row;
            if (m >= p.M) continue;
            float4 o = *reinterpret_cast<const float4*>(OUT + row * GC16_C + c4 * 4);
            if (bias) { const float4 bv = *reinterpret_cast<const float4*>(bias + c4 * 4); o.x += bv.x; o.y += bv.y; o.z += bv.z; o.w += bv.w; }
            if (p.act != ACT_NONE) { o.x = gc16_act(o.x, p.act); o.y = gc16_act(o.y, p.act); o.z = gc16_act(o.z, p.act); o.w = gc16_act(o.w, p.act); }
            const long gi = (long)m * p.out_rstride + c4 * 4;
            if constexpr (sizeof(TO) == 4) {
                if (rb) { const float4 rv = *reinterpret_cast<const float4*>(rb + gi); o.x += rv.x; o.y += rv.y; o.z += rv.z; o.w += rv.w; }
                *reinterpret_cast<float4*>(ob + gi) = o;
            } else {
                if (rb) { o.x += to_f32(rb[gi]); o.y += to_f32(rb[gi + 1]); o.z += to_f32(rb[gi + 2]); o.w += to_f32(rb[gi + 3]); }
                struct alignas(8) Q { TO a, b, c, d; };
                Q q; q.a = from_f32<TO>(o.x); q.b = from_f32<TO>(o.y); q.c = from_f32<TO>(o.z); q.d = from_f32<TO>(o.w);
                *reinterpret_cast<Q*>(ob + gi) = q;
            }
        }
    }
}


bool launch_gconv16(const ConvGemm& p, hipStream_t s) {
    const int odt = p.out_dtype < 0 ? p.dtype : p.out_dtype;
    if (!opt(OPT_GCONV16) || !p.gcp_w || (p.dtype != MI_F16 && p.dtype != MI_BF16) || (odt != p.dtype && odt != MI_F32)) return false;
    if (p.N != GC16_C || p.Cin != GC16_C || p.taps < 8 || p.taps > 127 || p.dil != 1) return false;
    if (p.epi != EPI_PLAIN || p.gate || p.accumulate || p.alpha != 1.f || p.out_planes || p.xp || p.ln_stats_in || p.ln_stats_out) return false;
    const int ev = odt == MI_F32 ? 4 : 4;
    if (p.x_rstride % 8 || p.x_bstride % 8 || p.x_goff % 8 || p.out_rstride % ev || p.out_bstride % ev) return false;
    if (((uintptr_t)p.x | (uintptr_t)p.gcp_w | (uintptr_t)p.out | (uintptr_t)p.res | (uintptr_t)p.bias) % 16) return false;
    if (p.pad < 0 || p.pad >= p.taps || p.M <= 0) return false;
    GConv16Dev d;
    d.x = p.x; d.img = p.gcp_w; d.bias = p.bias; d.out = p.out; d.res = p.res;
    d.T_in = p.T_in; d.M = p.M; d.taps = p.taps; d.pad = p.pad; d.act = p.act;
    d.x_bstride = p.x_bstride; d.x_rstride = p.x_rstride; d.x_goff = p.x_goff; d.out_bstride = p.out_bstride; d.out_rstride = p.out_rstride;
    constexpr int BM = 192;
    const int rows_a = BM + p.taps - 1;
    const size_t a_el = ((size_t)rows_a * GC16_S + 511) / 512 * 512;
    size_t lds = (a_el + (size_t)4 * GC16_WTAP) * 2;
    lds = std::max(lds, (size_t)BM * GC16_C * 4);
    if (lds > 80 * 1024) return false;
    const dim3 grid((p.M + BM - 1) / BM, p.G, p.B);
#define GC16_LAUNCH(T_, TO_)                                                                                                  \
    do {                                                                                                                      \
        auto kfn = gconv16_kernel<T_, TO_, BM>;                                                                               \
        MI_HIP(hipFuncSetAttribute((const void*)kfn, hipFuncAttributeMaxDynamicSharedMemorySize, 80 * 1024));                 \
        prof_set_kernel("gconv16_kernel<192> (16-bit grouped conv, weights as LDS images, two taps in flight)", "", "");      \
        hipLaunchKernelGGL(kfn, grid, dim3(512), lds, s, d);                                                                  \
    } while (0)
    if (p.dtype == MI_F16) { if (odt == MI_F32) GC16_LAUNCH(f16, float); else GC16_LAUNCH(f16, f16); }
    else { if (odt == MI_F32) GC16_LAUNCH(bf16, float); else GC16_LAUNCH(bf16, bf16); }
#undef GC16_LAUNCH
    MI_HIP(hipGetLastError());
    return true;
}

}
```

text-to-speech-tts-onnx_amd/csrc/gconv_pairs.hip:

```cpp
#include "common.h"
#include "gemm_epilogue.h"
#include "mfma.h"
#include "x3_split.h"
#include "lds_dma.h"

namespace mi {

struct GConvPairsDev {
    const float* x; const float* w; const float* bias; float* out; const float* res;
    int T_in, M, taps, pad, act;
    long x_bstride, x_rstride, x_goff, out_bstride, out_rstride;
    int K;
    int* sat;
};

constexpr int GCP_C = 64;
constexpr int GCP_S = GCP_C + 8;

__device__ __forceinline__ void gcp_split8(const float4 u, const float4 v, u32x4& hi, u32x4& lo, bool clamp) {
    const float f[8] = {u.x, u.y, u.z, u.w, v.x, v.y, v.z, v.w};
    unsigned h[4], l[4];
#pragma unroll
    for (int q = 0; q < 4; ++q) {
        if (clamp) x2_split_pair(f[2 * q], f[2 * q + 1], h[q], l[q]);
// ... 196 lines not shown
    {
        const int t_base = m0 - p.pad;
        const int nitem = rows_a * 8;
        unsigned sat = 0;
        for (int v = tid; v < nitem; v += 512) {
            const int row = v >> 3, c8 = v & 7;
            const int t = t_base + row;
            float4 u = float4{0.f, 0.f, 0.f, 0.f}, w2 = u;
            if (t >= 0 && t < p.T_in) {
                const float* src = xb + (long)t * p.x_rstride + c8 * 8;
                u = *reinterpret_cast<const float4*>(src);
                w2 = *reinterpret_cast<const float4*>(src + 4);
            }
            u32x4 h, l;
            gcp_split8(u, w2, h, l, true);
            sat |= x2_sat_word(h.x) | x2_sat_word(h.y) | x2_sat_word(h.z) | x2_sat_word(h.w);
            *reinterpret_cast<u32x4*>(AH + row * S + c8 * 8) = h;
            *reinterpret_cast<u32x4*>(AL + row * S + c8 * 8) = l;
        }
        sat_publish(p.sat, sat);
    }
    wait_vm<0>();
    __syncthreads();

    f32x16 acc[TM], accb[TM];
#pragma unroll
    for (int i = 0; i < TM; ++i)
#pragma unroll
        for (int r = 0; r < 16; ++r) { acc[i][r] = 0.f; accb[i][r] = 0.f; }
    for (int j = 0; j < npair; ++j) {
        if (j + 1 < npair) wdma(j + 1);
        const int t = 2 * j + kg;
        if (t < p.taps) {
            const f16* wt = WS + ((j & 1) * 2 + kg) * GCP_WTAP;
            const f16* bh_row = wt + (wn * 32 + lr) * S + hi * 8;
            const f16* bl_row = bh_row + GCP_C * S;
            const f16* ah_row = AH + (wm * WM + lr + t) * S + hi * 8;
            const f16* al_row = AL + (wm * WM + lr + t) * S + hi * 8;
#pragma unroll
            for (int ks = 0; ks < 4; ++ks) {
                const FH bh = *reinterpret_cast<const FH*>(bh_row + ks * 16);
                const FH bl = *reinterpret_cast<const FH*>(bl_row + ks * 16);
                FH ah[TM], al[TM];
#pragma unroll
                for (int i = 0; i < TM; ++i) {
                    ah[i] = *reinterpret_cast<const FH*>(ah_row + i * 32 * S + ks * 16);
                    al[i] = *reinterpret_cast<const FH*>(al_row + i * 32 * S + ks * 16);
                }
#pragma unroll
                for (int i = 0; i < TM; ++i) {
                    accb[i] = MH::mma(al[i], bh, accb[i]);
                    accb[i] = MH::mma(ah[i], bl, accb[i]);
                    acc[i] = MH::mma(ah[i], bh, acc[i]);
                }
            }
        }
        wait_vm<0>();
        __syncthreads();
    }
#pragma unroll
    for (int i = 0; i < TM; ++i)
#pragma unroll
        for (int r = 0; r < 16; ++r)
            OUT[(kg * BM + wm * WM + i * 32 + (r & 3) + 8 * (r >> 2) + 4 * hi) * GCP_C + wn * 32 + lr] = __builtin_fmaf(accb[i][r], 0x1p-11f, acc[i][r]);
    __syncthreads();
    {
        float* ob = p.out + (long)b * p.out_bstride + (long)g * GCP_C;
        const float* rb = p.res ? p.res + (long)b * p.out_bstride + (long)g * GCP_C : nullptr;
        const float* bias = p.bias ? p.bias + g * GCP_C : nullptr;
        for (int v = tid; v < BM * 16; v += 512) {
            const int row = v >> 4, c4 = v & 15;
            const int m = m0 + row;
            if (m >= p.M) continue;
            float4 o = *reinterpret_cast<const float4*>(OUT + row * GCP_C + c4 * 4);
            const float4 o1 = *reinterpret_cast<const float4*>(OUT + (BM + row) * GCP_C + c4 * 4);
            o.x += o1.x; o.y += o1.y; o.z += o1.z; o.w += o1.w;
            if (bias) { const float4 bv = *reinterpret_cast<const float4*>(bias + c4 * 4); o.x += bv.x; o.y += bv.y; o.z += bv.z; o.w += bv.w; }
            if (p.act != ACT_NONE) { o.x = gcp_act(o.x, p.act); o.y = gcp_act(o.y, p.act); o.z = gcp_act(o.z, p.act); o.w = gcp_act(o.w, p.act); }
            const long gi = (long)m * p.out_rstride + c4 * 4;
            if (rb) { const float4 rv = *reinterpret_cast<const float4*>(rb + gi); o.x += rv.x; o.y += rv.y; o.z += rv.z; o.w += rv.w; }
            *reinterpret_cast<float4*>(ob + gi) = o;
        }
    }
}


bool launch_gconv_pairs(const ConvGemm& p, hipStream_t s) {
    const int odt = p.out_dtype < 0 ? p.dtype : p.out_dtype;
    if (p.dtype != MI_F32 || odt != MI_F32 || p.N != GCP_C || p.Cin != GCP_C || p.taps < 8 || p.taps > 127 || p.dil != 1) return false;
    if (p.epi != EPI_PLAIN || p.gate || p.accumulate || p.alpha != 1.f || p.out_planes || p.xp) return false;
    if (p.x_rstride % 4 || p.x_bstride % 4 || p.x_goff % 4 || p.out_rstride % 4 || p.out_bstride % 4) return false;
    if (((uintptr_t)p.x | (uintptr_t)p.w | (uintptr_t)p.out | (uintptr_t)p.res | (uintptr_t)p.bias) % 16) return false;
    if (p.pad < 0 || p.pad >= p.taps || p.M <= 0) return false;
    GConvPairsDev d;
    d.x = (const float*)p.x; d.w = (const float*)p.w; d.bias = p.bias; d.out = (float*)p.out; d.res = (const float*)p.res;
    d.T_in = p.T_in; d.M = p.M; d.taps = p.taps; d.pad = p.pad; d.act = p.act;
    d.x_bstride = p.x_bstride; d.x_rstride = p.x_rstride; d.x_goff = p.x_goff; d.out_bstride = p.out_bstride; d.out_rstride = p.out_rstride;
    d.K = p.taps * GCP_C; d.sat = p.sat;
    const int cus = device_cus();
    auto load = [&](int bm) { const long n = (long)((p.M + bm - 1) / bm) * p.G * p.B; return ((n + cus - 1) / cus) * bm; };
    const int BM = load(192) < load(128) ? 192 : 128;
    const int rows_a = BM + p.taps - 1;
    size_t lds = ((size_t)2 * rows_a * GCP_S + (size_t)2 * GCP_C * GCP_S) * sizeof(f16);
    lds = std::max(lds, (size_t)BM * GCP_C * 4);
    lds = (lds + 15) / 16 * 16;
    if (lds > 160 * 1024) return false;
    const dim3 grid((p.M + BM - 1) / BM, p.G, p.B);
#define GCP_LAUNCH(BMv)                                                                                                       \
    do {                                                                                                                      \
        auto kfn = gconv_pairs_kernel<BMv>;                                                                                   \
         \
        if (lds > 64 * 1024) MI_HIP(hipFuncSetAttribute((const void*)kfn, hipFuncAttributeMaxDynamicSharedMemorySize, 160 * 1024)); \
        prof_set_kernel("gconv_pairs_kernel<" #BMv "> (fp32 grouped conv, fp16 pairs split once per workgroup)", "", "");      \
        hipLaunchKernelGGL(kfn, grid, dim3(256), lds, s, d);                                                                  \
    } while (0)
    if (p.gcp_w && opt(OPT_GCONV_TWO_TAPS)) {
        constexpr int BM2 = 192;
        const int ra = BM2 + p.taps - 1;
        const size_t a_el = ((size_t)ra * GCP_S + 511) / 512 * 512;
        size_t lds2 = (2 * a_el + (size_t)4 * GCP_WTAP) * sizeof(f16);
        lds2 = std::max(lds2, (size_t)2 * BM2 * GCP_C * 4);
        if (lds2 <= 160 * 1024) {
            auto kfn = gconv_pairs2_kernel<BM2>;
            MI_HIP(hipFuncSetAttribute((const void*)kfn, hipFuncAttributeMaxDynamicSharedMemorySize, 160 * 1024));
            prof_set_kernel("gconv_pairs2_kernel<192> (fp32 grouped conv, fp16 pairs, weights split at load, two taps in flight)", "", "");
            hipLaunchKernelGGL(kfn, dim3((p.M + BM2 - 1) / BM2, p.G, p.B), dim3(512), lds2, s, d, (const f16*)p.gcp_w);
            MI_HIP(hipGetLastError());
            return true;
        }
    }
    if (BM == 192) GCP_LAUNCH(192); else GCP_LAUNCH(128);
#undef GCP_LAUNCH
    MI_HIP(hipGetLastError());
    return true;
}

}
```

text-to-speech-tts-onnx_amd/csrc/options.h:

```cpp
#pragma once
#include <atomic>
#include <shared_mutex>

namespace mi {

#define MI_OPTIONS(X)                                                                                                   \
                                   \
    X(GEMM_BIG_TILE_MIN, "gemm_big_tile_min", "MI355TTS_BIG_TILE_MIN", ENV_INT, 160, STORE, 0, 0)                       \
    X(GEMM_N192_MIN, "gemm_n192_min", nullptr, ENV_INT, 160, STORE, 0, 0)                                               \
    X(GEMM_MID_TILE_MIN, "gemm_mid_tile_min", nullptr, ENV_INT, 160, STORE, 0, 0)                                       \
    X(GEMM_DMA3_K_MIN, "gemm_dma3_k_min", "MI355TTS_DMA3_K_MIN", ENV_INT, 2048, STORE, 0, 0)                            \
    X(GEMM_USE_DMA3, "gemm_use_dma3", "MI355TTS_NO_DMA3_GEMM", ENV_ONE_OFF, 1, BOOL, 0, 1)                              \
    X(GEMM_USE_DMA, "gemm_use_dma", "MI355TTS_NO_DMA_GEMM", ENV_ONE_OFF, 1, BOOL, 0, 1)                                 \
    X(GEMM_BIG_TILES, "gemm_big_tiles", "MI355TTS_NO_BIG_TILES", ENV_ONE_OFF, 1, BOOL, 0, 1)                            \
    X(GEMM_N192, "gemm_n192", "MI355TTS_NO_N192", ENV_ONE_OFF, 1, BOOL, 0, 1)                                           \
    X(GEMM_F32_DMA, "gemm_f32_dma", nullptr, ENV_INT, 1, BOOL, 0, 1)                                                    \
    X(GEMM_RING4, "gemm_ring4", "MI355TTS_NO_RING4", ENV_ONE_OFF, 1, BOOL, 0, 1)                                        \
    X(GEMM_RING4_MAX, "gemm_ring4_max", "MI355TTS_RING4_MAX", ENV_INT, 256, STORE, 0, 0)                                \
    X(GEMM_BUF, "gemm_buf", "MI355TTS_NO_BUF", ENV_ONE_OFF, 1, BOOL, 0, 1)                                              \
    X(GEMM_F32_SMALL, "gemm_f32_small", "MI355TTS_NO_F32_SMALL", ENV_ONE_OFF, 1, BOOL, 0, 1)                            \
    X(GEMM_F32_SMALL_MAX, "gemm_f32_small_max", "MI355TTS_F32_SMALL_MAX", ENV_INT, 1024, STORE, 0, 0)                   \
    X(GEMM_SMALL16_MAX, "gemm_small16_max", "MI355TTS_SMALL16_MAX", ENV_INT, 256, STORE, 0, 0)                          \
    X(GEMM_F32_N64_DMA, nullptr, "MI355TTS_F32_N64_DMA", ENV_INT, 1, STORE, 0, 0)                                       \
    X(GEMM_N64_DMA16, nullptr, "MI355TTS_N64_DMA16", ENV_INT, 0, STORE, 0, 0)  \
    X(GEMM_XCD_ORDER, nullptr, "MI355TTS_XCD_ORDER", ENV_ONE_ON, 0, BOOL, 0, 1)                                         \
    X(GEMM_LDS_EPI, nullptr, "MI355TTS_NO_LDS_EPI", ENV_ONE_OFF, 1, BOOL, 0, 1)                                         \
    X(GEMM_ROW_SPLIT, "gemm_row_split", nullptr, ENV_INT, 1, STORE, 0, 0)  \
     \
    X(GEMM_SK, "gemm_sk", "MI355TTS_SK", ENV_INT, 1, STORE, 0, 0)                                                       \
    X(GEMM_SK_STAGES, "gemm_sk_stages", "MI355TTS_SK_STAGES", ENV_INT, 0, STORE, 0, 0)                                  \
    X(GEMM_SK_ORDER, nullptr, "MI355TTS_SK_ORDER", ENV_INT, -1, STORE, 0, 0)                                            \
     \
     \
    X(GEMM_SK_QKV32, nullptr, "MI355TTS_SK_QKV32", ENV_INT, 0, STORE, 0, 0)                                             \
     \
    X(GEMM_F32_X3, "gemm_f32_x3", "MI355TTS_F32_X3", ENV_INT, 1, STORE, 0, 0)                                           \
    X(GEMM_F32_X3P, "gemm_f32_x3p", "MI355TTS_F32_X3P", ENV_INT, 1, STORE, 0, 0)                                        \
    X(GEMM_F32_PLANES, "gemm_f32_planes", "MI355TTS_F32_PLANES", ENV_INT, 2, REJECT, 2, 3)  \
    X(GEMM_F32_N64_PAIRS, "gemm_f32_n64_pairs", nullptr, ENV_INT, 1, STORE, 0, 0)  \
    X(GEMM_F32_GCONV, "gemm_f32_gconv", nullptr, ENV_INT, 1, STORE, 0, 0)  \
    X(GEMM_X3P_NOALIGN, "gemm_x3p_noalign", "MI355TTS_X3P_NOALIGN", ENV_INT, 0, STORE, 0, 0)  \
    X(GEMM_X3P_GRID, "gemm_x3p_grid", "MI355TTS_X3P_GRID", ENV_INT, 0, STORE, 0, 0)  \
    X(GEMM_X3D, "gemm_x3d", "MI355TTS_X3D", ENV_INT, 1, STORE, 0, 0)                            \
    X(GEMM_X3D_MIN_EFF, "gemm_x3d_min_eff", "MI355TTS_X3D_MIN_EFF", ENV_INT, 90, STORE, 0, 0)  \
     \
     \
     \
    X(EPI_WT, nullptr, "MI355TTS_EPI_WT", ENV_INT, 14, CLAMP, 0, 63)                                                    \
       \
    X(GEMM_PH8, "gemm_ph8", "MI355TTS_PH8", ENV_INT, 1, STORE, 0, 0)                                                    \
    X(GEMM_PH8_MIN_TILES, "gemm_ph8_min_tiles", "MI355TTS_PH8_MIN", ENV_INT, 200, STORE, 0, 0)                          \
    X(GEMM_PH8_ORDER, "gemm_ph8_order", "MI355TTS_PH8_ORDER", ENV_INT, 1, STORE, 0, 0)                                  \
     \
    X(GEMM_PH8_SPLIT_MAX, "gemm_ph8_split_max", "MI355TTS_PH8_SPLIT", ENV_INT, 2, CLAMP, 1, 4)                          \
    X(GEMM_PH8_SPLIT_MIN_NK, "gemm_ph8_split_min_nk", nullptr, ENV_INT, 24, STORE, 0, 0)                                \
                                                                            \
    X(GCONV_TWO_TAPS, "gconv_two_taps", "MI355TTS_GCONV2", ENV_ZERO_OFF, 1, BOOL, 0, 1)                                 \
    X(GCONV16, "gconv16", "MI355TTS_GCONV16", ENV_ZERO_OFF, 1, BOOL, 0, 1)                                              \
                                                                                         \
    X(ATTN_F32_X3, "attn_f32_x3", "MI355TTS_ATTN_X3", ENV_INT, 2, CLAMP, 0, 2)                                          \
    X(ATTN_F32_PLANES, "attn_f32_planes", "MI355TTS_ATTN_PLANES", ENV_INT, 2, REJECT, 2, 3)  \
    X(ATTN_SPLIT, "attn_split", "MI355TTS_ATTN_NO_SPLIT", ENV_ONE_OFF, 2, CLAMP, 0, 2)  \
    X(ATTN_XCD_MAP, "attn_xcd_map", nullptr, ENV_INT, 1, BOOL, 0, 1)  \
    X(ATTN_KV_PLANES, "attn_kv_planes", "MI355TTS_ATTN_KVP", ENV_INT, 1, BOOL, 0, 1)  \
    X(ATTN_V_ROWS, nullptr, "MI355TTS_ATTN_V_ROWS", ENV_ZERO_OFF, 1, BOOL, 0, 1)  \
    X(ATTN_LPT, "attn_lpt", "MI355TTS_ATTN_LPT", ENV_INT, 1, BOOL, 0, 1)  \
    X(ATTN_Z_FORCE, "attn_z_force", nullptr, ENV_INT, 0, CLAMP, 0, 4)  \
            \
    X(ATTN_Z, nullptr, "MI355TTS_ATTN_Z", ENV_INT, 4, CLAMP, 1, 4)                                                      \
    X(ATTN_Z16, nullptr, "MI355TTS_ATTN_Z16", ENV_INT, 1, CLAMP, 1, 4)                                                  \
    X(ATTN_CUTS, nullptr, "MI355TTS_ATTN_CUTS", ENV_CUTS, 0, STORE, 0, 0)  \
                                                                                              \
    X(GPT_MFMA_MIN, "gpt_mfma_min", nullptr, ENV_INT, 9, STORE, 0, 0)  \
    X(GPT_MFMA, nullptr, "MI355TTS_GPT_NO_MFMA", ENV_ONE_OFF, 1, BOOL, 0, 1)                                            \
                                                                    \
    X(BIGVGAN_STREAMS, "bigvgan_streams", nullptr, ENV_INT, 3, CLAMP, 1, 3)                                             \
    X(BV_SYNC, nullptr, "MI355TTS_BV_SYNC", ENV_ONE_ON, 0, BOOL, 0, 1)                                                  \
    X(AA_TILE, "aa_tile", "MI355TTS_AA_TILE", ENV_INT, 8192, STORE, 0, 0)    \
    X(AA_PIPE, "aa_pipe", "MI355TTS_AA_PIPE", ENV_ZERO_OFF, 1, BOOL, 0, 1)    \
    X(AA_R, "aa_r", "MI355TTS_AA_R", ENV_INT, 16, STORE, 0, 0)  \
    X(AACONV_LDS_MIN, "aaconv_lds_min", "MI355TTS_AACONV_LDS_MIN", ENV_INT, 0, STORE, 0, 0)

#define MI_OPT_ENUM(name, key, env, conv, dflt, policy, lo, hi) OPT_##name,
enum Opt : int { MI_OPTIONS(MI_OPT_ENUM) OPT_COUNT };

extern std::atomic<long> g_opt[OPT_COUNT];
static inline long opt(Opt o) { return g_opt[o].load(std::memory_order_relaxed); }

void options_init();
bool options_set(const char* key, long v);
bool options_get(const char* key, long* v);
struct AttnCuts { int n = 0; int c[3] = {0, 0, 0}; };
const AttnCuts& opt_attn_cuts();

long env_int(const char* name, long dflt);
bool env_first_is(const char* name, char c);

long option_epoch();
void option_epoch_bump();
std::shared_mutex& option_lock();
}
```

text-to-speech-tts-onnx_amd/mi355tts/_lib.py:

```python
from __future__ import annotations

import ctypes as C
import os

import numpy as np

MI_F32, MI_F16, MI_BF16 = 0, 1, 2
MI_HOST, MI_DEVICE = 0, 1
MI_EINVAL = -1
MI_ESTATE = -4
DTYPES = {"f32": MI_F32, "fp32": MI_F32, "float32": MI_F32, "f16": MI_F16, "fp16": MI_F16, "float16": MI_F16,
          "bf16": MI_BF16, "bfloat16": MI_BF16}

_LIB_PATH = os.environ.get("MI355TTS_LIB") or os.path.join(os.path.dirname(os.path.abspath(__file__)), "libmi355tts.so")
_lib = None


class MiError(RuntimeError):
    pass


def lib_path() -> str:
    return _LIB_PATH

# ... 98 lines not shown
    L.mi_gpt_text_embed.argtypes = [vp, vp, C.c_int, vp, C.c_int]; L.mi_gpt_text_embed.restype = C.c_int
    L.mi_gpt_mel_embed.argtypes = [vp, C.c_int32, C.c_int64, vp, C.c_int]; L.mi_gpt_mel_embed.restype = C.c_int
    L.mi_gpt_reset.argtypes = [vp]; L.mi_gpt_reset.restype = C.c_int
    L.mi_gpt_history_len.argtypes = [vp]; L.mi_gpt_history_len.restype = C.c_int64
    L.mi_gpt_step.argtypes = [vp, vp, C.c_int, vp, C.c_int, vp, vp, vp, C.c_int]; L.mi_gpt_step.restype = C.c_int
    L.mi_gpt_kv_read.argtypes = [vp, C.c_int, vp, vp, C.c_int]; L.mi_gpt_kv_read.restype = C.c_int
    L.mi_gpt_kv_write.argtypes = [vp, C.c_int, vp, vp, C.c_int, C.c_int]; L.mi_gpt_kv_write.restype = C.c_int
    L.mi_gpt_generate.argtypes = [vp, vp, C.c_int, C.c_int, vp, C.c_int, C.c_float, C.c_int, vp, vp, vp,
                                  C.POINTER(C.c_int32), C.c_int]
    L.mi_gpt_generate.restype = C.c_int
    L.mi_gpt_generate_batch.argtypes = [vp, C.c_int, vp, C.POINTER(C.c_int32), C.POINTER(C.c_int32), vp, C.c_int,
                                        C.c_float, C.c_int, vp, vp, vp, C.c_int, C.POINTER(C.c_int32), C.c_int]
    L.mi_gpt_generate_batch.restype = C.c_int
    L.mi_gpt_generate_sampled.argtypes = L.mi_gpt_generate.argtypes + [C.c_float, C.c_int, C.c_float, C.c_uint64]
    L.mi_gpt_generate_sampled.restype = C.c_int
    L.mi_gpt_generate_batch_sampled.argtypes = L.mi_gpt_generate_batch.argtypes + [vp, vp, vp, vp]
    L.mi_gpt_generate_batch_sampled.restype = C.c_int
    L.mi_gpt_generate_queue.argtypes = [vp, C.c_int, vp, C.POINTER(C.c_int32), C.POINTER(C.c_int32), vp, C.c_int, C.c_float,
                                        C.c_int, vp, vp, C.c_int, C.POINTER(C.c_int32), C.c_int, vp, vp, vp, vp, vp]
    L.mi_gpt_generate_queue.restype = C.c_int
    if hasattr(L, "mi_gpt_queue_begin"):
        L.mi_gpt_queue_begin.argtypes = [vp, C.c_int, vp, C.POINTER(C.c_int32), C.POINTER(C.c_int32), vp, C.c_int, C.c_float,
                                         C.c_int, vp, vp, C.c_int, C.c_int, vp, vp, vp, vp]
        L.mi_gpt_queue_begin.restype = C.c_int
        L.mi_gpt_queue_advance.argtypes = [vp, vp, vp, vp, vp]; L.mi_gpt_queue_advance.restype = C.c_int
        L.mi_gpt_queue_end.argtypes = [vp]; L.mi_gpt_queue_end.restype = C.c_int
    if hasattr(L, "mi_gpt_generate_queue_beam"):
        L.mi_gpt_generate_queue_beam.argtypes = [vp, C.c_int, vp, C.POINTER(C.c_int32), C.POINTER(C.c_int32), vp, C.c_int,
                                                 C.c_float, C.c_int, C.c_int, vp, vp, C.c_int, C.POINTER(C.c_int32), vp, C.c_int, vp]
        L.mi_gpt_generate_queue_beam.restype = C.c_int
        L.mi_gpt_queue_begin_beam.argtypes = [vp, C.c_int, vp, C.POINTER(C.c_int32), C.POINTER(C.c_int32), vp, C.c_int, C.c_float,
                                              C.c_int, C.c_int, vp, vp, C.c_int, vp, C.c_int]
        L.mi_gpt_queue_begin_beam.restype = C.c_int
    if hasattr(L, "mi_gpt_queue_schedule"):
        L.mi_gpt_queue_schedule.argtypes = [C.c_int, vp, vp, vp, C.c_int, C.c_int, C.c_int, vp, vp, vp, vp]
        L.mi_gpt_queue_schedule.restype = C.c_int
    L.mi_gpt_sample_logits.argtypes = [vp, vp, C.c_int, C.c_int, vp, vp, vp, vp, vp, vp, vp, vp, C.c_int]
    L.mi_gpt_sample_logits.restype = C.c_int
    L.mi_gpt_generate_beam.argtypes = [vp, C.c_int, vp, C.POINTER(C.c_int32), C.POINTER(C.c_int32), vp, C.c_int, C.c_float,
                                       C.c_int, vp, C.c_int, vp, vp, C.c_int, C.POINTER(C.c_int32), vp, C.c_int]
    L.mi_gpt_generate_beam.restype = C.c_int
    L.mi_gpt_beam_select.argtypes = [vp, vp, vp, C.c_int, C.c_int, C.c_int, C.c_int, vp, vp, vp, C.c_int]
    L.mi_gpt_beam_select.restype = C.c_int
    if hasattr(L, "mi_gpt_generate_beam_pool"):
        L.mi_gpt_generate_beam_pool.argtypes = [vp, C.c_int, vp, C.POINTER(C.c_int32), C.POINTER(C.c_int32), vp, C.c_int, C.c_float,
                                                C.c_int, vp, C.c_int, C.c_float, C.c_int, vp, vp, vp, vp, vp, vp, C.c_int,
                                                C.POINTER(C.c_int32), vp, C.c_int]
        L.mi_gpt_generate_beam_pool.restype = C.c_int
        L.mi_gpt_beam_pool_select.argtypes = [vp, vp, vp, C.c_int, C.c_int, C.c_int, C.c_int, vp, C.c_int, vp, vp, vp, C.c_float,
                                              C.c_int, vp, vp, vp, vp, vp, vp, vp, vp, vp, vp, vp, vp, C.c_int]
        L.mi_gpt_beam_pool_select.restype = C.c_int
    if hasattr(L, "mi_gpt_attn_decode"):
        L.mi_gpt_attn_decode.argtypes = [vp, vp, vp] + [C.c_int] * 4 + [vp, vp, C.c_int]
        L.mi_gpt_attn_decode.restype = C.c_int
        L.mi_gpt_attn_decode_beam.argtypes = [vp, vp, vp] + [C.c_int] * 4 + [vp, vp, C.c_int, vp, vp, C.c_int]
        L.mi_gpt_attn_decode_beam.restype = C.c_int
        L.mi_gpt_attn_prompt.argtypes = [vp, vp, vp] + [C.c_int] * 6 + [vp, C.c_int]
        L.mi_gpt_attn_prompt.restype = C.c_int
        L.mi_gpt_attn_prompt_packed.argtypes = [vp, vp, vp] + [C.c_int] * 4 + [vp, C.c_int, C.c_int, vp, C.c_int]
        L.mi_gpt_attn_prompt_packed.restype = C.c_int
    if hasattr(L, "mi_gpt_linear_decode"):
        L.mi_gpt_linear_decode.argtypes = [vp, vp, vp] + [C.c_int] * 3 + [vp] * 6 + [C.c_int] * 5 + [vp, vp, vp, C.c_int]
        L.mi_gpt_linear_decode.restype = C.c_int
        L.mi_gpt_linear_batch.argtypes = [vp, vp, vp, vp] + [C.c_int] * 4 + [vp] + [C.c_int] * 3 + [vp, C.c_int, vp, vp, vp, C.c_int]
        L.mi_gpt_linear_batch.restype = C.c_int
        L.mi_gpt_linear_batch_rows.argtypes = [C.c_int]
        L.mi_gpt_linear_batch_rows.restype = C.c_int
    if hasattr(L, "mi_gpt_create_q8"):
        L.mi_gpt_create_q8.argtypes = [C.POINTER(C.c_int32), C.c_int, vp, C.c_int64, C.c_int, C.c_int, C.c_int]
        L.mi_gpt_create_q8.restype = C.c_void_p
        L.mi_gpt_weight_bytes.argtypes = [vp]; L.mi_gpt_weight_bytes.restype = C.c_int64
        L.mi_gpt_quantize_u8.argtypes = [vp, C.c_int, C.c_int, vp, vp, vp]; L.mi_gpt_quantize_u8.restype = C.c_int
        L.mi_gpt_linear_decode_q8.argtypes = [vp, vp] + L.mi_gpt_linear_decode.argtypes
        L.mi_gpt_linear_decode_q8.restype = C.c_int
        L.mi_gpt_linear_batch_q8.argtypes = [vp, vp] + L.mi_gpt_linear_batch.argtypes
        L.mi_gpt_linear_batch_q8.restype = C.c_int
    L.mi_gpt_bench_pick.argtypes = [vp, C.c_int, C.c_int, vp, vp, vp, C.POINTER(C.c_double)]
    L.mi_gpt_bench_pick.restype = C.c_int
    L.mi_bench_conv_gemm.argtypes = [C.c_int] * 9 + [C.POINTER(C.c_double)]
    L.mi_bench_conv_gemm.restype = C.c_int
    if hasattr(L, "mi_conv_gemm_plan"):
        L.mi_conv_gemm_plan.argtypes = [C.c_int] * 9 + [C.POINTER(C.c_int32), C.POINTER(C.c_int)]
        L.mi_conv_gemm_plan.restype = C.c_int
    L.mi_set_option.argtypes = [C.c_char_p, C.c_int64]; L.mi_set_option.restype = C.c_int
    L.mi_get_option.argtypes = [C.c_char_p, C.POINTER(C.c_int64)]; L.mi_get_option.restype = C.c_int
    L.mi_device_pci_bus_id.argtypes = [C.c_int, C.c_char_p, C.c_int]; L.mi_device_pci_bus_id.restype = C.c_int
    L.mi_prof_enable.argtypes = [C.c_int]; L.mi_prof_enable.restype = C.c_int
    L.mi_prof_reset.argtypes = []; L.mi_prof_reset.restype = C.c_int
    L.mi_prof_get.argtypes = [C.c_char_p, C.POINTER(C.c_double), C.POINTER(C.c_int64), C.POINTER(C.c_double),
                              C.POINTER(C.c_double)]
    L.mi_prof_get.restype = C.c_int
    L.mi_prof_kernel_count.argtypes = []; L.mi_prof_kernel_count.restype = C.c_int
    L.mi_prof_kernel_get.argtypes = [C.c_int, C.c_char_p, C.c_int, C.c_char_p, C.c_int, C.POINTER(C.c_double), C.POINTER(C.c_int64),
                                     C.POINTER(C.c_double), C.POINTER(C.c_double)]
    L.mi_prof_kernel_get.restype = C.c_int
    _lib = L
    return L


def check(rc: int, what: str = "") -> None:
    if rc != 0:
        msg = load().mi_last_error().decode("utf-8", "replace")
        raise MiError(f"{what}: {msg} (code {rc})")


def f32p(a: np.ndarray):
    assert a.dtype == np.float32 and a.flags["C_CONTIGUOUS"]
    return a.ctypes.data_as(C.POINTER(C.c_float))


def i32p(a: np.ndarray):
    assert a.dtype == np.int32 and a.flags["C_CONTIGUOUS"]
    return a.ctypes.data_as(C.POINTER(C.c_int32))


def init(device: int = 0) -> None:
    check(load().mi_init(device), "mi_init")


PROF_FAMILIES = ("conv_gemm", "aa_act", "conv_post", "attn", "norm", "other")


def prof_enable(families=()) -> None:
    if families is True:
        mask = -1
    elif not families:
        mask = 0
    else:
        mask = 0
        for f in families:
            mask |= 1 << PROF_FAMILIES.index(f)
    load().mi_prof_enable(mask)


def prof_reset() -> None:
    check(load().mi_prof_reset(), "mi_prof_reset")


def prof_get(family: str) -> dict:
    ms, n, by, fl = C.c_double(), C.c_int64(), C.c_double(), C.c_double()
    check(load().mi_prof_get(family.encode(), C.byref(ms), C.byref(n), C.byref(by), C.byref(fl)), "mi_prof_get")
    return {"ms": ms.value, "launches": n.value, "bytes": by.value, "flops": fl.value}


def prof_kernels() -> list:
    L = load()
    out = []
    for i in range(L.mi_prof_kernel_count()):
        name, fam = C.create_string_buffer(256), C.create_string_buffer(32)
        ms, by, fl, n = C.c_double(0), C.c_double(0), C.c_double(0), C.c_int64(0)
        check(L.mi_prof_kernel_get(i, name, 256, fam, 32, C.byref(ms), C.byref(n), C.byref(by), C.byref(fl)), "mi_prof_kernel_get")
        out.append({"kernel": name.value.decode(), "family": fam.value.decode(), "ms": ms.value, "launches": int(n.value),
                    "bytes": by.value, "flops": fl.value})
    return sorted(out, key=lambda k: -k["ms"])


def bench_conv_gemm(dtype: str, B: int, T: int, Cin: int, N: int, taps: int = 1, dil: int = 1, with_res: bool = False,
                    iters: int = 20) -> float:
    ms = C.c_double()
    check(load().mi_bench_conv_gemm(DTYPES[dtype], B, T, Cin, N, taps, dil, int(with_res), iters, C.byref(ms)),
          "mi_bench_conv_gemm")
    return ms.value


GEMM_KINDS = ("none", "direct 256x32", "direct 128x64", "direct 128x128", "dma 64x64", "dma 64x64 fp16 pairs", "dma 128", "dma 128 ring4",
              "ph8", "x3p", "x3", "stream-k", "dma3 192", "dma3 256", "dma3 128")


def conv_gemm_plan(dtype: str, B: int, T: int, Cin: int, N: int, taps: int = 1, dil: int = 1, with_res: bool = False,
                   cus: int = 256) -> list:
    plans, n = (C.c_int32 * 20)(), C.c_int(0)
    check(load().mi_conv_gemm_plan(DTYPES.get(dtype, -1), B, T, Cin, N, taps, dil, int(with_res), cus, plans, C.byref(n)), "mi_conv_gemm_plan")
    keys = ("Tm", "Tn", "RT", "RC", "lds_epi", "use_buf")
    return [dict(zip(keys, plans[10 * i + 1:10 * i + 7]), kind=GEMM_KINDS[plans[10 * i]], grid=list(plans[10 * i + 7:10 * i + 10])) for i in range(n.value)]


def device_pci_bus_id(device: int) -> str:
    buf = C.create_string_buffer(64)
    check(load().mi_device_pci_bus_id(int(device), buf, 64), "mi_device_pci_bus_id")
    return buf.value.decode()


def set_option(key: str, value: int) -> None:
    check(load().mi_set_option(key.encode(), int(value)), "mi_set_option")


def get_option(key: str) -> int:
    v = C.c_int64(0)
    check(load().mi_get_option(key.encode(), C.byref(v)), "mi_get_option")
    return int(v.value)
```

Measured before the change: 44.31.

## Write noise panel planes in CFG update and add 144-row grouped conv kernel

The CFG update kernel now also writes the fp16 split panel planes of the next step's noise input. On later steps of a call, the DiT input projection can then skip the cat_noise and x3p split passes and reuse those planes. Separately, a grouped-conv pairs kernel with a 144-row tile and two taps in flight is selected when it balances work across CUs better than the 192-row tile. Both paths are on by default through new options. The cost is extra plane bookkeeping, a required invariant that the input projection stays on the plane kernel, and a new test entry point.

```diff
diff --git a/include/mi355tts.h b/include/mi355tts.h
--- a/include/mi355tts.h
+++ b/include/mi355tts.h
@@ -205,6 +205,9 @@
 int         mi_bench_conv_gemm(int dtype, int B, int T, int Cin, int N, int taps, int dil, int with_res, int iters,
                                double* ms);
 
+int         mi_gconv_pairs_unit(const float* x, const float* w, const float* bias, const float* res, float* out, int B, int T, int T_out,
+                                int G, int out_ld, int taps, int act, int img_G, int img_taps, float sentinel, int* rows_per_wg);
+
 #define MI_GEMM_PLAN_INTS 10
 int         mi_conv_gemm_plan(int dtype, int B, int T, int Cin, int N, int taps, int dil, int with_res, int cus,
                               int32_t* plans , int* n_launches);
diff --git a/text-to-speech-tts-onnx_amd/csrc/capi.hip b/text-to-speech-tts-onnx_amd/csrc/capi.hip
--- a/text-to-speech-tts-onnx_amd/csrc/capi.hip
+++ b/text-to-speech-tts-onnx_amd/csrc/capi.hip
@@ -324,6 +324,7 @@
         const std::string k(key);
         if (k == "f32_arithmetic") v = e.dtype != MI_F32 ? -1 : !gemm_x3_enabled() ? ARITH_NATIVE : (gemm_x3p_enabled() ? e.np : ARITH_BF16X3);
         else if (k == "saturation_events") v = e.sat_events;
+        else if (k == "noise_plane_updates") v = e.noise_plane_updates;
         else if (k == "adaln_fold") v = (e.fold_built && e.cfg.ln_fold != 0) ? 1 : 0;
         else if (k == "attn_v_rows") v = attention_kv_layout(0, e.dtype, true).v_rows;
         else MI_REQUIRE(false, "mi_f5_info: unknown key");
@@ -1584,6 +1585,37 @@
                              qkv, hist, max_seq, kc, vc, out, mem);
 }
 
+int mi_gconv_pairs_unit(const float* x, const float* w, const float* bias, const float* res, float* out, int B, int T, int T_out, int G,
+                        int out_ld, int taps, int act, int img_G, int img_taps, float sentinel, int* rows_per_wg) {
+    return guard([&] {
+        MI_REQUIRE(x && w && out && B > 0 && T > 0 && T_out >= T && G > 0 && out_ld >= G * 64 && out_ld % 4 == 0 && taps >= 8 && taps <= 127,
+                   "mi_gconv_pairs_unit: bad arguments");
+        hipStream_t s;
+        MI_HIP(hipStreamCreateWithFlags(&s, hipStreamNonBlocking));
+        struct Closer { hipStream_t s; ~Closer() { (void)hipStreamSynchronize(s); (void)hipStreamDestroy(s); } } closer{s};
+        const int C = G * 64;
+        const size_t nx = (size_t)B * T * C, nw = (size_t)C * taps * 64, no = (size_t)B * T_out * out_ld;
+        DevBuf dx, dw, db, dr, dout, img;
+        auto up = [&](DevBuf& d, const float* h, size_t n) { d.ensure(n * 4); MI_HIP(hipMemcpyAsync(d.p, h, n * 4, hipMemcpyHostToDevice, s)); };
+        up(dx, x, nx); up(dw, w, nw);
+        if (bias) up(db, bias, (size_t)C);
+        if (res) up(dr, res, no);
+        std::vector<float> fill(no, sentinel);
+        up(dout, fill.data(), no);
+        img.ensure(gconv_pairs_planes_bytes(G, taps));
+        gconv_pairs_split_weights(dw.as<float>(), img.p, G, taps, s);
+        ConvGemm g;
+        g.dtype = MI_F32; g.out_dtype = MI_F32; g.x = dx.p; g.w = dw.p; g.bias = db.as<float>(); g.out = dout.p; g.res = dr.p;
+        g.B = B; g.G = G; g.T_in = T; g.M = T; g.N = 64; g.Cin = 64; g.taps = taps; g.pad = taps / 2;
+        g.x_bstride = (long)T * C; g.x_rstride = C; g.x_goff = 64; g.out_bstride = (long)T_out * out_ld; g.out_rstride = out_ld;
+        g.act = act ? ACT_MISH : ACT_NONE; g.gcp_w = img.p; g.gcp_G = img_G; g.gcp_taps = img_taps;
+        if (rows_per_wg) *rows_per_wg = gconv_pairs_rows(g, device_cus());
+        launch_conv_gemm(g, s);
+        MI_HIP(hipMemcpyAsync(out, dout.p, no * 4, hipMemcpyDeviceToHost, s));
+        MI_HIP(hipStreamSynchronize(s));
+    });
+}
+
 extern "C++" {
 enum { BG_X, BG_W, BG_BIAS, BG_OUT, BG_RES, BG_W3, BG_XP, BG_W3P, BG_SK_WS, BG_SK_FLAGS, BG_COUNT };
 template <typename F> static ConvGemm bench_gemm(int dtype, int B, int T, int Cin, int N, int taps, int dil, int with_res, F&& buf) {
diff --git a/text-to-speech-tts-onnx_amd/csrc/common.h b/text-to-speech-tts-onnx_amd/csrc/common.h
--- a/text-to-speech-tts-onnx_amd/csrc/common.h
+++ b/text-to-speech-tts-onnx_amd/csrc/common.h
@@ -144,6 +144,7 @@
     const void* w3 = nullptr;
     const void* xp = nullptr; const void* w3p = nullptr; int np = 3;
     const void* gcp_w = nullptr;
+    int gcp_G = 0, gcp_taps = 0;
     void* out_planes = nullptr;
     const float* ln_scale = nullptr; void* ln_out = nullptr; float* ln_stats_out = nullptr; int ln_out_np = 0;
     const float* ln_stats_in = nullptr; const float* ln_p = nullptr; const float* ln_c = nullptr; int ln_dim = 0; float ln_eps = 0.f;
@@ -179,6 +180,7 @@
 void x3p_split_rows(const float* x, long ld, void* planes, int rows, int K, hipStream_t s, int np = 3, int* sat = nullptr);
 size_t gconv_pairs_planes_bytes(int G, int taps);
 void gconv_pairs_split_weights(const float* w, void* wp, int G, int taps, hipStream_t s);
+int gconv_pairs_rows(const ConvGemm& p, int cus);
 size_t gconv16_image_bytes(int G, int taps);
 void gconv16_build_weights(const void* w, int dtype, void* img, int G, int taps, hipStream_t s);
 int x3p_planes();
diff --git a/text-to-speech-tts-onnx_amd/csrc/f5.h b/text-to-speech-tts-onnx_amd/csrc/f5.h
--- a/text-to-speech-tts-onnx_amd/csrc/f5.h
+++ b/text-to-speech-tts-onnx_amd/csrc/f5.h
@@ -52,7 +52,7 @@
     struct VBlock { DevBuf dw_w, dw_b, n_w, n_b; Lin pw1, pw2; };
     std::vector<VBlock> vblocks;
 
-    struct GraphEntry { hipGraphExec_t exec = nullptr; int uses = 0; };
+    struct GraphEntry { hipGraphExec_t exec = nullptr; int uses = 0; long plane_updates = 0; };
     std::map<std::vector<int>, GraphEntry> graphs;
     bool use_graph = true;
     long graph_epoch = 0;
@@ -69,6 +69,9 @@
     int arith_kind = ARITH_DEFAULT;
     DevBuf Ap, Ap2;
     int ap2_cols() const { return std::max(cfg.ff(), cat_ld()); }
+    DevBuf ApIn;
+    bool in_planes_live = false;
+    long noise_plane_updates = 0;
     bool fold_built = false;
     DevBuf ApN;
     DevBuf ln_stats;
@@ -89,15 +92,16 @@
     F5(const F5Cfg& c, const float* w, int64_t nw, int dt, int dev, int mem = MI_HOST);
     ~F5();
     void ensure_workspace(int U, int N);
-    void gemm(int dt, const void* x, long xb, long xr, int K, const Lin& L, void* out, int odt, long ob, long orr,
-              int B, int M, int act = ACT_NONE, const void* res = nullptr, const float* gate = nullptr);
+    bool gemm(int dt, const void* x, long xb, long xr, int K, const Lin& L, void* out, int odt, long ob, long orr,
+              int B, int M, int act = ACT_NONE, const void* res = nullptr, const float* gate = nullptr, DevBuf* planes = nullptr,
+              bool split = true);
     int preprocess(int U, const int16_t* audio, long L, const int32_t* text_ids, int T, int N,
                    const float* noise_in, uint64_t seed, int mem);
     void stft(const int16_t* audio_dev, int U, long L, int pad = -1);
     void check_text_ids();
     void load_cond(const float* noise, const float* cmt, const float* cmtd, int U, int N, int mem);
     void build_cat_cond(int U, int N);
-    void dit_eval(int U, int N, int k, const int* lens = nullptr);
+    void dit_eval(int U, int N, int k, const int* lens = nullptr, bool first = true);
     void steps(int U, int N, int k0, int nsteps, const int* lens = nullptr);
     DevBuf d_len;
     std::vector<int> h_len;
diff --git a/text-to-speech-tts-onnx_amd/csrc/f5.hip b/text-to-speech-tts-onnx_amd/csrc/f5.hip
--- a/text-to-speech-tts-onnx_amd/csrc/f5.hip
+++ b/text-to-speech-tts-onnx_amd/csrc/f5.hip
@@ -408,7 +408,9 @@
     if (ws_U > 0) {
         const long rows = (long)2 * ws_U * ws_N;
         Ap.ensure((size_t)x3p_bytes(rows, cfg.dim, np)); Ap2.ensure((size_t)x3p_bytes(rows, ap2_cols(), np)); ApN.ensure((size_t)x3p_bytes(rows, cfg.dim, np));
-    }
+        ApIn.ensure((size_t)x3p_bytes(rows, cat_ld(), np));
+    }
+    in_planes_live = false;
     MI_HIP(hipStreamSynchronize(stream));
 }
 
@@ -484,6 +486,7 @@
     if (dtype == MI_F32) {
         Ap.ensure((size_t)x3p_bytes((long)rows, c.dim, np)); Ap2.ensure((size_t)x3p_bytes((long)rows, ap2_cols(), np));
         if (fold_built) ApN.ensure((size_t)x3p_bytes((long)rows, c.dim, np));
+        ApIn.ensure((size_t)x3p_bytes((long)rows, cat_ld(), np));
     }
     if (fold_built) { ln_stats.ensure((rows + 128) * (size_t)(c.dim / LN_BLK) * 2 * 4); if (dtype != MI_F32) ln_fin.ensure((rows + 128) * 8); }
     pred.ensure(rows * c.mel * 4 * proj_parts);
@@ -499,8 +502,8 @@
     ws_U = Um; ws_N = Nm;
 }
 
-void F5::gemm(int dt, const void* x, long xb, long xr, int K, const Lin& L, void* out, int odt, long ob, long orr, int B,
-              int M, int act, const void* res, const float* gate) {
+bool F5::gemm(int dt, const void* x, long xb, long xr, int K, const Lin& L, void* out, int odt, long ob, long orr, int B,
+              int M, int act, const void* res, const float* gate, DevBuf* planes, bool split) {
     ConvGemm g;
     g.dtype = dt; g.out_dtype = odt; g.x = x; g.w = L.w.p; g.w3 = L.w3.p; g.bias = L.b.p ? L.b.as<float>() : nullptr; g.out = out;
     g.res = res; g.gate = gate; g.gate_bstride = 0;
@@ -512,16 +515,17 @@
         g.B = 1; g.T_in = B * M; g.M = B * M;
     }
     if (dt == MI_F32 && L.w3p.p && g.B == 1 && Ap.p && gemm_x3p_enabled()) {
-        DevBuf& ab = K <= cfg.dim ? Ap : Ap2;
+        DevBuf& ab = planes ? *planes : K <= cfg.dim ? Ap : Ap2;
         g.xp = ab.p; g.w3p = L.w3p.p; g.np = np;
-        if (gemm_x3p_would_run(g, device_cus())) {
+        if (ab.p && gemm_x3p_would_run(g, device_cus())) {
             MI_REQUIRE(x3p_bytes(g.M, K, np) <= (long)ab.bytes, "F5::gemm: the panel planes of the rows do not fit their buffer");
-            x3p_split_rows((const float*)x, xr, const_cast<void*>(g.xp), g.M, K, stream, np, d_sat.as<int>());
+            if (split) x3p_split_rows((const float*)x, xr, const_cast<void*>(g.xp), g.M, K, stream, np, d_sat.as<int>());
         } else {
             g.xp = nullptr; g.w3p = nullptr;
         }
     }
     launch_conv_gemm(g, stream);
+    return g.xp != nullptr;
 }
 
 static inline uint64_t splitmix64(uint64_t x) {
@@ -657,15 +661,19 @@
         }
 }
 
-void F5::dit_eval(int U, int N, int k, const int* lens) {
+void F5::dit_eval(int U, int N, int k, const int* lens, bool first) {
     const F5Cfg& c = cfg;
     MI_REQUIRE(k >= 0 && k < c.nfe, "f5: time step out of range");
     hipStream_t s = stream;
     const int B = 2 * U, d = c.dim, ld = cat_ld(), ff = c.ff(), H = c.heads, D = c.dim_head;
     const long rows = (long)B * N;
     const float* modk = mod.as<float>() + (size_t)k * mod_ld;
-    launch_cat_noise(d_noise.as<float>(), cat.p, U, N, c.mel, ld, dtype, s);
-    gemm(dtype, cat.p, (long)N * ld, ld, ld, in_proj, h32.p, MI_F32, (long)N * d, d, B, N);
+    const bool noise_planes = opt(OPT_NOISE_PLANES) != 0;
+    const bool keep = noise_planes && !first && in_planes_live;
+    if (!keep) launch_cat_noise(d_noise.as<float>(), cat.p, U, N, c.mel, ld, dtype, s);
+    const bool on_planes = gemm(dtype, cat.p, (long)N * ld, ld, ld, in_proj, h32.p, MI_F32, (long)N * d, d, B, N, ACT_NONE, nullptr, nullptr, &ApIn, !keep);
+    MI_REQUIRE(!keep || on_planes, "f5: the input projection left the panel-plane kernel between two evaluations of a call");
+    in_planes_live = noise_planes && on_planes;
     const void* hin = h32.p;
     if (dtype != MI_F32) { launch_copy2d(h32.as<float>(), d, hT.p, d, rows, d, dtype, s); hin = hT.p; }
     const long row_bytes = (long)d * (long)dtype_size(dtype);
@@ -675,7 +683,7 @@
         g.dtype = dtype; g.x = hin; g.w = gconv1.w.p; g.bias = gconv1.b.as<float>(); g.out = c1.p;
         g.B = B; g.G = c.pos_g; g.T_in = N; g.M = N; g.N = d / c.pos_g; g.Cin = d / c.pos_g; g.taps = c.pos_k; g.pad = c.pos_k / 2;
         g.x_bstride = (long)N * d; g.x_rstride = d; g.x_goff = d / c.pos_g; g.out_bstride = (long)N * d; g.out_rstride = d;
-        g.act = ACT_MISH; g.sat = d_sat.as<int>(); g.gcp_w = gconv1.w3p.p;
+        g.act = ACT_MISH; g.sat = d_sat.as<int>(); g.gcp_w = gconv1.w3p.p; g.gcp_G = c.pos_g; g.gcp_taps = c.pos_k;
         launch_conv_gemm(g, s);
         if (lens) launch_zero_pad_rows(c1.p, row_bytes, B, N, lens, 2, s);
         g.x = c1.p; g.w = gconv2.w.p; g.bias = gconv2.b.as<float>(); g.out = X.p; g.out_dtype = MI_F32; g.res = h32.p; g.gcp_w = gconv2.w3p.p;
@@ -813,12 +821,18 @@
 
 void F5::steps_eager(int U, int N, int k0, int nsteps, const int* lens) {
     for (int k = k0; k < k0 + nsteps; ++k) {
-        dit_eval(U, N, k, lens);
+        dit_eval(U, N, k, lens, k == k0);
+        NoisePlanes np_out;
+        if (in_planes_live && k + 1 < k0 + nsteps) {
+            np_out.planes = ApIn.p; np_out.nch = cat_ld() >> 5; np_out.np = np; np_out.sat = d_sat.as<int>();
+            ++noise_plane_updates;
+        }
         if (lens)
             launch_cfg_update_len(d_noise.as<float>(), pred.as<float>(), U, N, cfg.mel, cfg.cfg_strength, delta_t.as<float>(), k, lens, stream,
-                                  proj_parts);
+                                  proj_parts, np_out);
         else
-            launch_cfg_update(d_noise.as<float>(), pred.as<float>(), U, N, cfg.mel, cfg.cfg_strength, delta_t.as<float>(), k, stream, proj_parts);
+            launch_cfg_update(d_noise.as<float>(), pred.as<float>(), U, N, cfg.mel, cfg.cfg_strength, delta_t.as<float>(), k, stream, proj_parts,
+                              np_out);
     }
 }
 
@@ -848,9 +862,10 @@
     if (!use_graph || prof_mask() != 0 || nsteps < 2) { steps_eager(U, N, k0, nsteps, lens); return; }
     if (graph_epoch != option_epoch()) { drop_graphs(); graph_epoch = option_epoch(); }
     GraphEntry& e = graphs[{U, N, k0, nsteps, lens ? 1 : 0}];
-    if (e.exec) { MI_HIP(hipGraphLaunch(e.exec, stream)); return; }
+    if (e.exec) { MI_HIP(hipGraphLaunch(e.exec, stream)); noise_plane_updates += e.plane_updates; return; }
     if (e.uses++ == 0) { steps_eager(U, N, k0, nsteps, lens); return; }
     hipGraph_t graph = nullptr;
+    const long updates_before = noise_plane_updates;
     MI_HIP(hipStreamBeginCapture(stream, hipStreamCaptureModeThreadLocal));
     try {
         steps_eager(U, N, k0, nsteps, lens);
@@ -862,7 +877,8 @@
     MI_HIP(hipStreamEndCapture(stream, &graph));
     hipError_t err = hipGraphInstantiate(&e.exec, graph, nullptr, nullptr, 0);
     (void)hipGraphDestroy(graph);
-    if (err != hipSuccess) { e.exec = nullptr; use_graph = false; steps_eager(U, N, k0, nsteps, lens); return; }
+    e.plane_updates = noise_plane_updates - updates_before;
+    if (err != hipSuccess) { e.exec = nullptr; use_graph = false; noise_plane_updates = updates_before; steps_eager(U, N, k0, nsteps, lens); return; }
     MI_HIP(hipGraphLaunch(e.exec, stream));
 }
 
diff --git a/text-to-speech-tts-onnx_amd/csrc/f5_kernels.h b/text-to-speech-tts-onnx_amd/csrc/f5_kernels.h
--- a/text-to-speech-tts-onnx_amd/csrc/f5_kernels.h
+++ b/text-to-speech-tts-onnx_amd/csrc/f5_kernels.h
@@ -29,9 +29,11 @@
 void launch_istft_ola(const float* frames, const float* wsi, int U, int F, int nfft, int hop, float* out_f,
                       int16_t* out_i, hipStream_t s);
 void launch_cat_noise(const float* noise, void* cat, int U, int N, int M, int ldc, int dtype, hipStream_t s);
-void launch_cfg_update(float* noise, const float* pred, int U, int N, int M, float cfg, const float* dt, int k, hipStream_t s, int parts = 1);
+struct NoisePlanes { void* planes = nullptr; int nch = 0, np = 2; int* sat = nullptr; };
+void launch_cfg_update(float* noise, const float* pred, int U, int N, int M, float cfg, const float* dt, int k, hipStream_t s, int parts = 1,
+                       const NoisePlanes& out = NoisePlanes());
 void launch_cfg_update_len(float* noise, const float* pred, int U, int N, int M, float cfg, const float* dt, int k, const int* len,
-                           hipStream_t s, int parts = 1);
+                           hipStream_t s, int parts = 1, const NoisePlanes& out = NoisePlanes());
 void launch_zero_pad_rows(void* x, long row_bytes, int items, int N, const int* len, int per, hipStream_t s);
 void launch_sum_parts(const float* in, float* out, long rows, int M, int parts, hipStream_t s);
 
diff --git a/text-to-speech-tts-onnx_amd/csrc/f5_kernels.hip b/text-to-speech-tts-onnx_amd/csrc/f5_kernels.hip
--- a/text-to-speech-tts-onnx_amd/csrc/f5_kernels.hip
+++ b/text-to-speech-tts-onnx_amd/csrc/f5_kernels.hip
@@ -591,44 +591,65 @@
     MI_HIP(hipGetLastError());
 }
 
+template <int NP>
+__device__ __forceinline__ void noise_to_planes(float v, unsigned char* __restrict__ planes, long u, long n, int N, int m, int nch, unsigned& sat) {
+    unsigned w[NP];
+    if constexpr (NP == 3) x3_split_pair(v, 0.f, w[0], w[1], w[2]);
+    else { x2_split_pair(v, 0.f, w[0], w[1]); sat |= x2_sat_word(w[0]); }
+#pragma unroll
+    for (int br = 0; br < 2; ++br) {
+        unsigned char* dst = planes + x3p_slot_offset((2 * u + br) * N + n, m >> 3, nch, NP) + (m & 7) * 2;
+#pragma unroll
+        for (int q = 0; q < NP; ++q) *reinterpret_cast<unsigned short*>(dst + q * X3P_PLANE) = (unsigned short)(w[q] & 0xffffu);
+    }
+}
+template <int NP, bool LEN>
 __global__ __launch_bounds__(256) void cfg_update_kernel(float* __restrict__ noise, const float* __restrict__ pred,
-                                                         long NM, int M, int parts, long total, float cfg, const float* __restrict__ dt, int k) {
+                                                         long NM, int M, int parts, long total, float cfg, const float* __restrict__ dt, int k,
+                                                         const int* __restrict__ len, unsigned char* __restrict__ planes, int nch,
+                                                         int* __restrict__ satp) {
     const long i = (long)blockIdx.x * 256 + threadIdx.x;
     if (i >= total) return;
     const long u = i / NM, r = i - u * NM;
     const long n = r / M; const int m = (int)(r - n * M);
-    const float* c = pred + ((2 * u) * NM + n * M) * parts + m;
-    const float* un = c + NM * parts;
-    float pc = c[0], pu = un[0];
-    for (int q = 1; q < parts; ++q) { pc += c[(long)q * M]; pu += un[(long)q * M]; }
-    noise[i] += (pc + (pc - pu) * cfg) * dt[k];
-}
-void launch_cfg_update(float* noise, const float* pred, int U, int N, int M, float cfg, const float* dt, int k, hipStream_t s, int parts) {
+    float v = 0.f;
+    if (!LEN || n < len[u]) {
+        const float* c = pred + ((2 * u) * NM + n * M) * parts + m;
+        const float* un = c + NM * parts;
+        float pc = c[0], pu = un[0];
+        for (int q = 1; q < parts; ++q) { pc += c[(long)q * M]; pu += un[(long)q * M]; }
+        v = noise[i] + (pc + (pc - pu) * cfg) * dt[k];
+    }
+    noise[i] = v;
+    if constexpr (NP != 0) {
+        unsigned sat = 0;
+        noise_to_planes<NP>(v, planes, u, n, (int)(NM / M), m, nch, sat);
+        if constexpr (NP == 2) sat_publish(satp, sat);
+    }
+}
+template <bool LEN>
+static void launch_cfg_update_any(float* noise, const float* pred, int U, int N, int M, float cfg, const float* dt, int k, const int* len,
+                                  hipStream_t s, int parts, const NoisePlanes& out) {
     const long total = (long)U * N * M;
-    hipLaunchKernelGGL(cfg_update_kernel, dim3((unsigned)((total + 255) / 256)), dim3(256), 0, s, noise, pred, (long)N * M, M, parts, total, cfg, dt, k);
-    MI_HIP(hipGetLastError());
-}
-
-__global__ __launch_bounds__(256) void cfg_update_len_kernel(float* __restrict__ noise, const float* __restrict__ pred,
-                                                             long NM, int M, int parts, long total, float cfg, const float* __restrict__ dt,
-                                                             int k, const int* __restrict__ len) {
-    const long i = (long)blockIdx.x * 256 + threadIdx.x;
-    if (i >= total) return;
-    const long u = i / NM, r = i - u * NM;
-    const long n = r / M; const int m = (int)(r - n * M);
-    if (n >= len[u]) { noise[i] = 0.f; return; }
-    const float* c = pred + ((2 * u) * NM + n * M) * parts + m;
-    const float* un = c + NM * parts;
-    float pc = c[0], pu = un[0];
-    for (int q = 1; q < parts; ++q) { pc += c[(long)q * M]; pu += un[(long)q * M]; }
-    noise[i] += (pc + (pc - pu) * cfg) * dt[k];
+    const dim3 grid((unsigned)((total + 255) / 256));
+    MI_REQUIRE(!out.planes || ((out.np == 2 || out.np == 3) && out.nch * 32 >= M), "cfg_update: bad noise planes");
+    const int np = out.planes ? out.np : 0;
+    auto go = [&](auto kern) {
+        hipLaunchKernelGGL(kern, grid, dim3(256), 0, s, noise, pred, (long)N * M, M, parts, total, cfg, dt, k, len, (unsigned char*)out.planes,
+                           out.nch, out.sat);
+    };
+    if (np == 2) go(cfg_update_kernel<2, LEN>);
+    else if (np == 3) go(cfg_update_kernel<3, LEN>);
+    else go(cfg_update_kernel<0, LEN>);
+    MI_HIP(hipGetLastError());
+}
+void launch_cfg_update(float* noise, const float* pred, int U, int N, int M, float cfg, const float* dt, int k, hipStream_t s, int parts,
+                       const NoisePlanes& out) {
+    launch_cfg_update_any<false>(noise, pred, U, N, M, cfg, dt, k, nullptr, s, parts, out);
 }
 void launch_cfg_update_len(float* noise, const float* pred, int U, int N, int M, float cfg, const float* dt, int k, const int* len,
-                           hipStream_t s, int parts) {
-    const long total = (long)U * N * M;
-    hipLaunchKernelGGL(cfg_update_len_kernel, dim3((unsigned)((total + 255) / 256)), dim3(256), 0, s, noise, pred, (long)N * M, M, parts,
-                       total, cfg, dt, k, len);
-    MI_HIP(hipGetLastError());
+                           hipStream_t s, int parts, const NoisePlanes& out) {
+    launch_cfg_update_any<true>(noise, pred, U, N, M, cfg, dt, k, len, s, parts, out);
 }
 
 __global__ __launch_bounds__(256) void zero_pad_rows_kernel(uint4* __restrict__ x, int row_vec, int N, const int* __restrict__ len, int per) {
diff --git a/text-to-speech-tts-onnx_amd/csrc/gconv16.hip b/text-to-speech-tts-onnx_amd/csrc/gconv16.hip
--- a/text-to-speech-tts-onnx_amd/csrc/gconv16.hip
+++ b/text-to-speech-tts-onnx_amd/csrc/gconv16.hip
@@ -165,6 +165,7 @@
     if (p.x_rstride % 8 || p.x_bstride % 8 || p.x_goff % 8 || p.out_rstride % ev || p.out_bstride % ev) return false;
     if (((uintptr_t)p.x | (uintptr_t)p.gcp_w | (uintptr_t)p.out | (uintptr_t)p.res | (uintptr_t)p.bias) % 16) return false;
     if (p.pad < 0 || p.pad >= p.taps || p.M <= 0) return false;
+    MI_REQUIRE(p.gcp_G == p.G && p.gcp_taps == p.taps, "gconv16: the weight image was built for another group or tap count");
     GConv16Dev d;
     d.x = p.x; d.img = p.gcp_w; d.bias = p.bias; d.out = p.out; d.res = p.res;
     d.T_in = p.T_in; d.M = p.M; d.taps = p.taps; d.pad = p.pad; d.act = p.act;
diff --git a/text-to-speech-tts-onnx_amd/csrc/gconv_pairs.hip b/text-to-speech-tts-onnx_amd/csrc/gconv_pairs.hip
--- a/text-to-speech-tts-onnx_amd/csrc/gconv_pairs.hip
+++ b/text-to-speech-tts-onnx_amd/csrc/gconv_pairs.hip
@@ -302,6 +302,146 @@
             *reinterpret_cast<float4*>(ob + gi) = o;
         }
     }
+}
+
+constexpr int GCP3_BM = 144;
+constexpr int GCP3_SA = GCP_C + 16;
+
+typedef float gcp_f32x4 __attribute__((ext_vector_type(4)));
+
+template <>
+__global__ __launch_bounds__(768, 1) void gconv_pairs2_kernel<GCP3_BM>(const GConvPairsDev p, const f16* __restrict__ wplanes) {
+    using FH = f16x8;
+    constexpr int BM = GCP3_BM, S = GCP_S, SA = GCP3_SA, MB = 3, NB = 2;
+    extern __shared__ __attribute__((aligned(1024))) unsigned char smem_raw[];
+    const int rows_a = BM + p.taps - 1;
+    const int a_el = ((rows_a * SA + 511) / 512) * 512;
+    f16* AH = reinterpret_cast<f16*>(smem_raw);
+    f16* AL = AH + a_el;
+    f16* WS = AL + a_el;
+    float* OUT = reinterpret_cast<float*>(smem_raw);
+
+    const int tid = threadIdx.x, lane = tid & 63, fi = lane & 15, fs = lane >> 4;
+    const int wave = __builtin_amdgcn_readfirstlane(tid >> 6);
+    const int kg = wave / 6, w6 = wave - kg * 6, wm = w6 >> 1, wn = w6 & 1;
+    const int m0 = blockIdx.x * BM, g = blockIdx.y, b = blockIdx.z;
+    const float* xb = p.x + (long)b * p.x_bstride + (long)g * p.x_goff;
+    const int tp = (p.taps + 1) & ~1, npair = tp >> 1;
+    const f16* wg = wplanes + (long)g * tp * GCP_WTAP;
+
+    constexpr int NPIECE = 2 * GCP_WTAP * (int)sizeof(f16) / 1024;
+    static_assert(NPIECE % 12 == 0, "a tap pair is whole 1 KB pieces, the same number for every wave");
+    auto wdma = [&](int pair) {
+        const char* src = reinterpret_cast<const char*>(wg + (long)pair * 2 * GCP_WTAP) + lane * 16;
+        char* dst = reinterpret_cast<char*>(WS + (pair & 1) * 2 * GCP_WTAP);
+        for (int pc = wave; pc < NPIECE; pc += 12)
+            __builtin_amdgcn_global_load_lds((const __attribute__((address_space(1))) void*)(src + pc * 1024), (lds_void*)(dst + pc * 1024), 16, 0, 0);
+    };
+    wdma(0);
+    {
+        const int t_base = m0 - p.pad;
+        const int nitem = rows_a * 8;
+        unsigned sat = 0;
+        for (int v = tid; v < nitem; v += 768) {
+            const int row = v >> 3, c8 = v & 7;
+            const int t = t_base + row;
+            float4 u = float4{0.f, 0.f, 0.f, 0.f}, w2 = u;
+            if (t >= 0 && t < p.T_in) {
+                const float* src = xb + (long)t * p.x_rstride + c8 * 8;
+                u = *reinterpret_cast<const float4*>(src);
+                w2 = *reinterpret_cast<const float4*>(src + 4);
+            }
+            u32x4 h, l;
+            gcp_split8(u, w2, h, l, true);
+            sat |= x2_sat_word(h.x) | x2_sat_word(h.y) | x2_sat_word(h.z) | x2_sat_word(h.w);
+            *reinterpret_cast<u32x4*>(AH + row * SA + c8 * 8) = h;
+            *reinterpret_cast<u32x4*>(AL + row * SA + c8 * 8) = l;
+        }
+        sat_publish(p.sat, sat);
+    }
+    wait_vm<0>();
+    __syncthreads();
+
+    gcp_f32x4 acc[MB][NB], accb[MB][NB];
+#pragma unroll
+    for (int i = 0; i < MB; ++i)
+#pragma unroll
+        for (int j = 0; j < NB; ++j) { acc[i][j] = gcp_f32x4{0.f, 0.f, 0.f, 0.f}; accb[i][j] = gcp_f32x4{0.f, 0.f, 0.f, 0.f}; }
+    const int pcol = fi < 4 ? fi : fi >= 12 ? fi - 8 : fi + 4;
+    const int a_lane = (wm * 48 + fi) * SA + fs * 8;
+    const int b_lane = (wn * 32 + 2 * pcol) * S + fs * 8;
+    for (int j = 0; j < npair; ++j) {
+        if (j + 1 < npair) wdma(j + 1);
+        const int t = 2 * j + kg;
+        if (t < p.taps) {
+            const f16* bh_row = WS + ((j & 1) * 2 + kg) * GCP_WTAP + b_lane;
+            const f16* bl_row = bh_row + GCP_C * S;
+            const f16* ah_row = AH + t * SA + a_lane;
+            const f16* al_row = AL + t * SA + a_lane;
+#pragma unroll
+            for (int ks = 0; ks < 2; ++ks) {
+                FH ah[MB], al[MB], bh[NB], bl[NB];
+#pragma unroll
+                for (int i = 0; i < MB; ++i) al[i] = *reinterpret_cast<const FH*>(al_row + i * 16 * SA + ks * 32);
+#pragma unroll
+                for (int jb = 0; jb < NB; ++jb) bh[jb] = *reinterpret_cast<const FH*>(bh_row + jb * S + ks * 32);
+#pragma unroll
+                for (int i = 0; i < MB; ++i) ah[i] = *reinterpret_cast<const FH*>(ah_row + i * 16 * SA + ks * 32);
+#pragma unroll
+                for (int jb = 0; jb < NB; ++jb) bl[jb] = *reinterpret_cast<const FH*>(bl_row + jb * S + ks * 32);
+#pragma unroll
+                for (int i = 0; i < MB; ++i)
+#pragma unroll
+                    for (int jb = 0; jb < NB; ++jb) accb[i][jb] = __builtin_amdgcn_mfma_f32_16x16x32_f16(al[i], bh[jb], accb[i][jb], 0, 0, 0);
+#pragma unroll
+                for (int i = 0; i < MB; ++i)
+#pragma unroll
+                    for (int jb = 0; jb < NB; ++jb) accb[i][jb] = __builtin_amdgcn_mfma_f32_16x16x32_f16(ah[i], bl[jb], accb[i][jb], 0, 0, 0);
+#pragma unroll
+                for (int i = 0; i < MB; ++i)
+#pragma unroll
+                    for (int jb = 0; jb < NB; ++jb) acc[i][jb] = __builtin_amdgcn_mfma_f32_16x16x32_f16(ah[i], bh[jb], acc[i][jb], 0, 0, 0);
+            }
+        }
+        wait_vm<0>();
+        __syncthreads();
+    }
+#pragma unroll
+    for (int i = 0; i < MB; ++i)
+#pragma unroll
+        for (int jb = 0; jb < NB; ++jb)
+#pragma unroll
+            for (int r = 0; r < 4; ++r)
+                OUT[(kg * BM + wm * 48 + i * 16 + 4 * fs + r) * GCP_C + wn * 32 + 2 * pcol + jb] = __builtin_fmaf(accb[i][jb][r], 0x1p-11f, acc[i][jb][r]);
+    __syncthreads();
+    {
+        float* ob = p.out + (long)b * p.out_bstride + (long)g * GCP_C;
+        const float* rb = p.res ? p.res + (long)b * p.out_bstride + (long)g * GCP_C : nullptr;
+        const float* bias = p.bias ? p.bias + g * GCP_C : nullptr;
+        for (int v = tid; v < BM * 16; v += 768) {
+            const int row = v >> 4, c4 = v & 15;
+            const int m = m0 + row;
+            if (m >= p.M) continue;
+            float4 o = *reinterpret_cast<const float4*>(OUT + row * GCP_C + c4 * 4);
+            const float4 o1 = *reinterpret_cast<const float4*>(OUT + (BM + row) * GCP_C + c4 * 4);
+            o.x += o1.x; o.y += o1.y; o.z += o1.z; o.w += o1.w;
+            if (bias) { const float4 bv = *reinterpret_cast<const float4*>(bias + c4 * 4); o.x += bv.x; o.y += bv.y; o.z += bv.z; o.w += bv.w; }
+            if (p.act != ACT_NONE) { o.x = gcp_act(o.x, p.act); o.y = gcp_act(o.y, p.act); o.z = gcp_act(o.z, p.act); o.w = gcp_act(o.w, p.act); }
+            const long gi = (long)m * p.out_rstride + c4 * 4;
+            if (rb) { const float4 rv = *reinterpret_cast<const float4*>(rb + gi); o.x += rv.x; o.y += rv.y; o.z += rv.z; o.w += rv.w; }
+            *reinterpret_cast<float4*>(ob + gi) = o;
+        }
+    }
+}
+
+static size_t gcp_image_lds(int BM, int taps) {
+    const int ra = BM + taps - 1;
+    const size_t a_el = ((size_t)ra * (BM == GCP3_BM ? GCP3_SA : GCP_S) + 511) / 512 * 512;
+    return std::max((2 * a_el + (size_t)4 * GCP_WTAP) * sizeof(f16), (size_t)2 * BM * GCP_C * 4);
+}
+int gconv_pairs_rows(const ConvGemm& p, int cus) {
+    auto load = [&](int bm) { const long n = (long)((p.M + bm - 1) / bm) * p.G * p.B; return ((n + cus - 1) / cus) * bm; };
+    return opt(OPT_GCONV_EXACT) && gcp_image_lds(GCP3_BM, p.taps) <= 160 * 1024 && load(GCP3_BM) < load(192) ? GCP3_BM : 192;
 }
 
 
@@ -335,11 +475,17 @@
         hipLaunchKernelGGL(kfn, grid, dim3(256), lds, s, d);                                                                  \
     } while (0)
     if (p.gcp_w && opt(OPT_GCONV_TWO_TAPS)) {
+        MI_REQUIRE(p.gcp_G == p.G && p.gcp_taps == p.taps, "gconv_pairs: the weight image was built for another group or tap count");
+        if (gconv_pairs_rows(p, cus) == GCP3_BM) {
+            auto kfn = gconv_pairs2_kernel<GCP3_BM>;
+            MI_HIP(hipFuncSetAttribute((const void*)kfn, hipFuncAttributeMaxDynamicSharedMemorySize, 160 * 1024));
+            prof_set_kernel("gconv_pairs2_kernel<144> (fp32 grouped conv, fp16 pairs, weights split at load, two taps in flight, 16x16x32 blocks)", "", "");
+            hipLaunchKernelGGL(kfn, dim3((p.M + GCP3_BM - 1) / GCP3_BM, p.G, p.B), dim3(768), gcp_image_lds(GCP3_BM, p.taps), s, d, (const f16*)p.gcp_w);
+            MI_HIP(hipGetLastError());
+            return true;
+        }
         constexpr int BM2 = 192;
-        const int ra = BM2 + p.taps - 1;
-        const size_t a_el = ((size_t)ra * GCP_S + 511) / 512 * 512;
-        size_t lds2 = (2 * a_el + (size_t)4 * GCP_WTAP) * sizeof(f16);
-        lds2 = std::max(lds2, (size_t)2 * BM2 * GCP_C * 4);
+        const size_t lds2 = gcp_image_lds(BM2, p.taps);
         if (lds2 <= 160 * 1024) {
             auto kfn = gconv_pairs2_kernel<BM2>;
             MI_HIP(hipFuncSetAttribute((const void*)kfn, hipFuncAttributeMaxDynamicSharedMemorySize, 160 * 1024));
diff --git a/text-to-speech-tts-onnx_amd/csrc/options.h b/text-to-speech-tts-onnx_amd/csrc/options.h
--- a/text-to-speech-tts-onnx_amd/csrc/options.h
+++ b/text-to-speech-tts-onnx_amd/csrc/options.h
@@ -57,6 +57,10 @@
                                                                             \
     X(GCONV_TWO_TAPS, "gconv_two_taps", "MI355TTS_GCONV2", ENV_ZERO_OFF, 1, BOOL, 0, 1)                                 \
     X(GCONV16, "gconv16", "MI355TTS_GCONV16", ENV_ZERO_OFF, 1, BOOL, 0, 1)                                              \
+     \
+    X(GCONV_EXACT, nullptr, "MI355TTS_GCONV_EXACT", ENV_ZERO_OFF, 1, BOOL, 0, 1)                                        \
+     \
+    X(NOISE_PLANES, nullptr, "MI355TTS_NOISE_PLANES", ENV_ZERO_OFF, 1, BOOL, 0, 1)  \
                                                                                          \
     X(ATTN_F32_X3, "attn_f32_x3", "MI355TTS_ATTN_X3", ENV_INT, 2, CLAMP, 0, 2)                                          \
     X(ATTN_F32_PLANES, "attn_f32_planes", "MI355TTS_ATTN_PLANES", ENV_INT, 2, REJECT, 2, 3)  \
diff --git a/text-to-speech-tts-onnx_amd/mi355tts/_lib.py b/text-to-speech-tts-onnx_amd/mi355tts/_lib.py
--- a/text-to-speech-tts-onnx_amd/mi355tts/_lib.py
+++ b/text-to-speech-tts-onnx_amd/mi355tts/_lib.py
@@ -204,6 +204,9 @@
     if hasattr(L, "mi_conv_gemm_plan"):
         L.mi_conv_gemm_plan.argtypes = [C.c_int] * 9 + [C.POINTER(C.c_int32), C.POINTER(C.c_int)]
         L.mi_conv_gemm_plan.restype = C.c_int
+    if hasattr(L, "mi_gconv_pairs_unit"):
+        L.mi_gconv_pairs_unit.argtypes = [vp] * 5 + [C.c_int] * 9 + [C.c_float, C.POINTER(C.c_int)]
+        L.mi_gconv_pairs_unit.restype = C.c_int
     L.mi_set_option.argtypes = [C.c_char_p, C.c_int64]; L.mi_set_option.restype = C.c_int
     L.mi_get_option.argtypes = [C.c_char_p, C.POINTER(C.c_int64)]; L.mi_get_option.restype = C.c_int
     L.mi_device_pci_bus_id.argtypes = [C.c_int, C.c_char_p, C.c_int]; L.mi_device_pci_bus_id.restype = C.c_int
@@ -297,6 +300,24 @@
     return [dict(zip(keys, plans[10 * i + 1:10 * i + 7]), kind=GEMM_KINDS[plans[10 * i]], grid=list(plans[10 * i + 7:10 * i + 10])) for i in range(n.value)]
 
 
+def gconv_pairs_unit(x: np.ndarray, w: np.ndarray, bias=None, res=None, taps: int = 31, mish: bool = True, t_out: int = 0, out_ld: int = 0,
+                     image=None, sentinel: float = -7.0):
+    B, T, Cc = x.shape
+    G = Cc // 64
+    t_out, out_ld = t_out or T, out_ld or Cc
+    out = np.empty((B, t_out, out_ld), np.float32)
+    rows = C.c_int(0)
+    ig, it = image or (G, taps)
+    x, w = np.ascontiguousarray(x, np.float32), np.ascontiguousarray(w, np.float32)
+    bias = None if bias is None else np.ascontiguousarray(bias, np.float32)
+    res = None if res is None else np.ascontiguousarray(res, np.float32)
+    assert w.shape == (Cc, taps, 64) and (res is None or res.shape == out.shape)
+    vp = lambda a: None if a is None else a.ctypes.data_as(C.c_void_p)
+    check(load().mi_gconv_pairs_unit(vp(x), vp(w), vp(bias), vp(res), vp(out), B, T, t_out, G, out_ld, taps, int(mish), ig, it,
+                                     float(sentinel), C.byref(rows)), "mi_gconv_pairs_unit")
+    return out, rows.value
+
+
 def device_pci_bus_id(device: int) -> str:
     buf = C.create_string_buffer(64)
     check(load().mi_device_pci_bus_id(int(device), buf, 64), "mi_device_pci_bus_id")
```

Result: no change. 44.47, median of 6 (+0.4%).
